# AdamBeedell/MLX8-WS-Audio-Transformer

Hardware: AMD Instinct MI355X
Metric: 4s@16kHz clips/sec through mel+Whisper-small encoder (higher is better)
Workload: dtype fp16; 1 GPU; int16 PCM [B,64000] in HBM -> Whisper log-mel [B,80,3000] -> Whisper-small encoder -> hidden [B,1500,768] fp32; mode=parity (clip zero-padded to 30 s, as the reference computes), precision=f16f8, fp16_exact_projection_matrices=0 of 48 (found by the library at upload), parallelism=dp1 (clip shards, no data-path collective)

## Files before the change

mlx8-ws-audio-transformer_amd/build.py:

```python
from __future__ import annotations

import os
import subprocess
import sys
from concurrent.futures import ThreadPoolExecutor

HERE = os.path.dirname(os.path.abspath(__file__))
CSRC = os.path.join(HERE, "csrc")
OBJ = os.path.join(CSRC, "_obj")
LIB = os.path.join(HERE, "libawt.so")
SOURCES = ["awt_api.hip", "logmel.hip", "gemm.hip", "attention.hip", "attention_f8.hip", "attention_bwd.hip", "elementwise.hip", "comm.hip", "decoder_ops.hip", "decoder_grad.hip", "bmm.hip", "decode_select.hip", "alignment.hip", "wgrad.hip", "cnn_ops.hip"]
HIPCC = os.environ.get("HIPCC", "/opt/rocm/bin/hipcc")
FLAGS = ["--offload-arch=gfx950", "-O3", "-std=c++20", "-fPIC", "-fno-gpu-rdc", "-Wall", "-Wno-unused-function"]


def _stale(target: str, deps) -> bool:
    if not os.path.exists(target):
        return True
    t = os.path.getmtime(target)
    return any(os.path.getmtime(d) > t for d in deps)


def _compile(src: str, force: bool) -> str:
    obj = os.path.join(OBJ, src.replace(".hip", ".o"))
    deps = [os.path.join(CSRC, src), os.path.join(CSRC, "common.h"), os.path.join(CSRC, "comm.h"), os.path.join(CSRC, "gemm_pp.h"), os.path.join(CSRC, "wgrad.h"), os.path.join(HERE, "..", "include", "awt.h")]
    if force or _stale(obj, deps):
        cmd = [HIPCC, *FLAGS, "-c", os.path.join(CSRC, src), "-o", obj]
        r = subprocess.run(cmd, capture_output=True, text=True)
        if r.returncode != 0:
            raise RuntimeError(f"hipcc failed for {src}:\n{r.stdout}\n{r.stderr}")
        if r.stderr.strip():
            sys.stderr.write(r.stderr)
    return obj


def build(force: bool = False, verbose: bool = True) -> str:
    os.makedirs(OBJ, exist_ok=True)
    with ThreadPoolExecutor(max_workers=min(len(SOURCES), os.cpu_count() or 4)) as ex:
        objs = list(ex.map(lambda s: _compile(s, force), SOURCES))
    if force or _stale(LIB, objs):
        cmd = [HIPCC, "--offload-arch=gfx950", "-shared", "-fPIC", "-o", LIB, *objs, "-ldl"]
        r = subprocess.run(cmd, capture_output=True, text=True)
        if r.returncode != 0:
            raise RuntimeError(f"link failed:\n{r.stdout}\n{r.stderr}")
    if verbose:
        print(f"built {LIB}")
    return LIB


if __name__ == "__main__":
    build(force="--force" in sys.argv)
```

mlx8-ws-audio-transformer_amd/csrc/awt_api.hip:

```cpp
#include <string.h>
#include <algorithm>
#include <string>
#include <vector>

#include "common.h"
#include "comm.h"
#include "wgrad.h"

static thread_local std::string g_err;
void awt_set_error(const std::string& msg) { g_err = msg; }
int awt_fail(int code, const std::string& msg) { g_err = msg; return code; }
extern "C" const char* awt_last_error(void) { return g_err.c_str(); }
extern "C" const char* awt_version(void) { return "awt 0.1 (gfx950)"; }

struct awt_prof_state {
  struct Span { hipEvent_t a, b; };
  std::vector<Span> spans[AWT_PROF_NCLASSES];
  std::vector<Span> pool;
  double flops[AWT_PROF_NCLASSES] = {};
  Span open[AWT_PROF_NCLASSES];
};

void awt_prof_begin(awt_ctx* c, int klass, hipStream_t s, double flops) {
  awt_prof_state* p = c->prof;
  awt_prof_state::Span sp;
  if (!p->pool.empty()) { sp = p->pool.back(); p->pool.pop_back(); }
  else { (void)hipEventCreate(&sp.a); (void)hipEventCreate(&sp.b); }
  (void)hipEventRecord(sp.a, s);
  p->open[klass] = sp;
  p->flops[klass] += flops;
}
void awt_prof_end(awt_ctx* c, int klass, hipStream_t s) {
  awt_prof_state* p = c->prof;
  (void)hipEventRecord(p->open[klass].b, s);
  p->spans[klass].push_back(p->open[klass]);
}

static int g_conv_live = 1;
static int g_pp_mask = 12;
extern "C" int awt_tuning_set(const char* key, int value) {
  AWT_REQUIRE(key, AWT_ERR_INVALID, "tuning_set: null key");
  if (!strcmp(key, "gemm_tile")) {
    AWT_REQUIRE(value == 0 || value == 64 || value == 128 || value == 256, AWT_ERR_INVALID, "tuning_set: gemm_tile must be 0 (auto), 64, 128 or 256");
    awt_gemm_force_tile(value);
    return AWT_OK;
  }
  if (!strcmp(key, "gemm_gm")) {
    AWT_REQUIRE(value >= 0 && value <= 64, AWT_ERR_INVALID, "tuning_set: gemm_gm must be 0 (default) .. 64");
    awt_gemm_set_gm(value);
    return AWT_OK;
  }
  if (!strcmp(key, "gemm_pp")) {
    AWT_REQUIRE(value >= 0 && value <= 2, AWT_ERR_INVALID, "tuning_set: gemm_pp must be 0 (off), 1 (automatic, default) or 2 (wherever supported)");
    awt_gemm_set_pp_mode(value);
    return AWT_OK;
  }
  if (!strcmp(key, "gemm_pp_mask")) {
    AWT_REQUIRE(value >= 0 && value <= 15, AWT_ERR_INVALID, "tuning_set: gemm_pp_mask is a bit set 0 .. 15 (1 qkv, 2 out_proj, 4 fc1, 8 fc2; fc2 only together with fc1)");
    g_pp_mask = value;
    return AWT_OK;
  }
  if (!strcmp(key, "gemm_mfma16")) {
    AWT_REQUIRE(value == 0 || value == 1, AWT_ERR_INVALID, "tuning_set: gemm_mfma16 must be 1 (default: the f16f8 GEMM's 16 x 16 MFMA form where it applies) or 0 (32 x 32 only)");
    awt_gemm_set_mfma16(value);
    return AWT_OK;
  }
  if (!strcmp(key, "conv_live")) {
    AWT_REQUIRE(value == 0 || value == 1, AWT_ERR_INVALID, "tuning_set: conv_live must be 1 (default: the conv stem of awt_audio_encode computes the live positions only) or 0 (every position)");
    g_conv_live = value;
    return AWT_OK;
  }
  if (!strcmp(key, "attn_shape")) {
    AWT_REQUIRE(value == 0 || (value >= 4 && value <= 6), AWT_ERR_INVALID, "tuning_set: attn_shape must be 0 (auto), 4, 5 or 6");
    awt_attn_force_shape(value);
    return AWT_OK;
  }
  if (!strcmp(key, "attn_qt")) {
    AWT_REQUIRE(value >= 0 && value <= 2, AWT_ERR_INVALID, "tuning_set: attn_qt must be 0 (auto), 1 or 2");
    awt_attn_force_qt(value);
    return AWT_OK;
  }
  AWT_REQUIRE(false, AWT_ERR_INVALID, "tuning_set: unknown key");
}

extern "C" int awt_prof_enable(awt_ctx* c, int on) {
  AWT_REQUIRE(c, AWT_ERR_INVALID, "prof_enable: null ctx");
  if (!c->prof) c->prof = new awt_prof_state();
  c->prof_on = on;
  return AWT_OK;
}
extern "C" int awt_prof_collect(awt_ctx* c, int klass, double* total_ms, int64_t* launches, double* flops) {
  AWT_REQUIRE(c && c->prof && klass >= 0 && klass < AWT_PROF_NCLASSES, AWT_ERR_INVALID, "prof_collect: bad argument");
  awt_prof_state* p = c->prof;
  double ms = 0;
  for (auto& sp : p->spans[klass]) {
    AWT_HIP_CHECK(hipEventSynchronize(sp.b));
    float t = 0;
    AWT_HIP_CHECK(hipEventElapsedTime(&t, sp.a, sp.b));
    ms += t;
    p->pool.push_back(sp);
  }
  if (total_ms) *total_ms = ms;
  if (launches) *launches = (int64_t)p->spans[klass].size();
  if (flops) *flops = p->flops[klass];
  p->spans[klass].clear();
  p->flops[klass] = 0;
  return AWT_OK;
}

extern "C" int awt_ctx_create(int device, awt_ctx** out) {
  AWT_REQUIRE(out, AWT_ERR_INVALID, "ctx_create: null out");
  int n = 0;
  AWT_HIP_CHECK(hipGetDeviceCount(&n));
  AWT_REQUIRE(device >= 0 && device < n, AWT_ERR_INVALID, "ctx_create: no such device");
  AWT_HIP_CHECK(hipSetDevice(device));
  hipDeviceProp_t prop;
  AWT_HIP_CHECK(hipGetDeviceProperties(&prop, device));
  AWT_REQUIRE(strncmp(prop.gcnArchName, "gfx950", 6) == 0, AWT_ERR_INVALID,
              std::string("libawt is built for gfx950 (MI355X) only; device is ") + prop.gcnArchName);
  awt_ctx* c = new awt_ctx();
  c->device = device;
  if (hipMalloc(&c->zeros, 256) != hipSuccess || hipMemset(c->zeros, 0, 256) != hipSuccess) {
    delete c;
    AWT_REQUIRE(false, AWT_ERR_HIP, "ctx_create: could not allocate the zero page");
  }
  int rc = logmel_prepare_impl(c, 400, 80, 0.0, 8000.0, 16000, 1);
  if (!rc) rc = logmel_prepare_impl(c, 400, 128, 0.0, 8000.0, 16000, 1);
  if (rc) { awt_ctx_destroy(c); return rc; }
  *out = c;
  return AWT_OK;
}
extern "C" int awt_logmel_prepare(awt_ctx* c, int n_fft, int n_mels, float f_min, float f_max, int sample_rate, int slaney) {
  return logmel_prepare_impl(c, n_fft, n_mels, (double)f_min, (double)f_max, sample_rate, slaney);
}
extern "C" int awt_resample_prepare(awt_ctx* c, int sr_in, int sr_out) { return resample_prepare_impl(c, sr_in, sr_out); }
extern "C" void awt_ctx_destroy(awt_ctx* c) {
  if (!c) return;
  awt_free_tables(c);
  if (c->zeros) (void)hipFree(c->zeros);
  if (c->prof) {
    for (int k = 0; k < AWT_PROF_NCLASSES; ++k)
      for (auto& sp : c->prof->spans[k]) { (void)hipEventDestroy(sp.a); (void)hipEventDestroy(sp.b); }
    for (auto& sp : c->prof->pool) { (void)hipEventDestroy(sp.a); (void)hipEventDestroy(sp.b); }
    delete c->prof;
  }
  delete c;
}

extern "C" int awt_logmel_whisper(awt_ctx* c, const void* pcm, int pcm_is_i16, int64_t pcm_stride, const int32_t* n_valid,
                                  int max_valid, int B, int n_frames_out, float* out, void* workspace, size_t ws_bytes,
                                  void* stream) {
  return logmel_whisper_impl(c, pcm, pcm_is_i16, pcm_stride, n_valid, max_valid, B, n_frames_out, 80, out, workspace, ws_bytes,
                             (hipStream_t)stream);
}
extern "C" int awt_logmel_whisper_mels(awt_ctx* c, const void* pcm, int pcm_is_i16, int64_t pcm_stride, const int32_t* n_valid,
                                       int max_valid, int B, int n_frames_out, int n_mels, float* out, void* workspace, size_t ws_bytes,
                                       void* stream) {
  return logmel_whisper_impl(c, pcm, pcm_is_i16, pcm_stride, n_valid, max_valid, B, n_frames_out, n_mels, out, workspace, ws_bytes,
                             (hipStream_t)stream);
}
extern "C" int awt_logmel_whisper_signal(awt_ctx* c, const void* pcm, int pcm_is_i16, int64_t pcm_stride, const int32_t* n_valid,
                                         int max_valid, int B, int n_signal, int n_mels, float* out, void* workspace, size_t ws_bytes,
                                         void* stream) {
  return logmel_whisper_impl(c, pcm, pcm_is_i16, pcm_stride, n_valid, max_valid, B, 0, n_mels, out, workspace, ws_bytes, (hipStream_t)stream,
                             n_signal);
}
extern "C" int awt_logmel_generic(awt_ctx* c, const float* pcm, int64_t pcm_stride, int B, int n_samples, int sample_rate,
                                  int n_fft, int hop, int n_mels, float f_min, float f_max, float log_eps, float* out,
                                  void* stream) {
  return logmel_generic_impl(c, pcm, pcm_stride, B, n_samples, sample_rate, n_fft, hop, n_mels, f_min, f_max, log_eps, out,
                             (hipStream_t)stream);
}

extern "C" int64_t awt_resampled_length(int n_in, int sr_in, int sr_out) {
  if (n_in <= 0 || sr_in <= 0 || sr_out <= 0) return 0;
  return resampled_length(n_in, sr_in, sr_out);
}
extern "C" int awt_prepare_waveform(awt_ctx* c, const void* pcm, int pcm_is_i16, int channels, int64_t channel_stride,
                                    int64_t sample_stride, int n_in, int sr_in, int sr_out, float* out, int n_out, void* stream) {
  return prepare_waveform_impl(c, pcm, pcm_is_i16, channels, channel_stride, sample_stride, n_in, sr_in, sr_out, out, n_out,
                               (hipStream_t)stream);
}

namespace {

struct Planes {
  bf16_t* hi = nullptr; bf16_t* lo = nullptr; uint8_t* x8 = nullptr; int64_t rows = 0, ld = 0;
  int* d_inexact = nullptr; bool exact16 = false;
  int64_t s_rows = 0;
  bf16_t* s16 = nullptr; uint8_t* s8 = nullptr;
  char* pp = nullptr;
};
struct Linear {
  Planes w; float* bias = nullptr; int N = 0, K = 0;
};
struct LoraGroup {
  bool active = false;
  Planes a;
  Planes b;
  Planes bT;
  Planes aT;
  int kp = 0;
};
struct Layer {
  Linear qkv, out, fc1, fc2;
  Planes qkvT, outT, fc1T, fc2T;
  Planes fc1T8, fc2T8;
  Planes fc1_8, fc2_8;
  float *ln1_g = nullptr, *ln1_b = nullptr, *ln2_g = nullptr, *ln2_b = nullptr;
  LoraGroup lq, lo_, l1, l2;
};

int conv1_k(int n_mels) { return (3 * n_mels + 63) / 64 * 64; }

}

struct awt_encoder {
  awt_ctx* ctx = nullptr;
  awt_encoder_cfg cfg{};
  int planes = 1;
  int prec = PREC_BF16X3;
  Linear conv1, conv2;
  float* pos = nullptr;
  float* zero_row = nullptr;
  float *lnf_g = nullptr, *lnf_b = nullptr;
  std::vector<Layer> layers;
  std::vector<void*> allocs;
  std::vector<std::string> seen;
  int chunk = 16;
  awt_comm* comm = nullptr;
  int comm_groups = 2;
  bool mlp_f8 = false;
  float* wt_tmp = nullptr;
  int grad_scale_log2 = 0;
  bool train_base = false;
  Planes conv2T[3];
  struct GradEntry { std::string name; size_t offset; int64_t shape[3]; int rank; };
  std::vector<GradEntry> glayout;
  size_t g_head = 0, g_per_layer = 0;
};

namespace {

int dev_alloc(awt_encoder* e, void** p, size_t bytes) {
  AWT_HIP_CHECK(hipMalloc(p, bytes));
  AWT_HIP_CHECK(hipMemset(*p, 0, bytes));
  e->allocs.push_back(*p);
  return AWT_OK;
}
int alloc_planes(awt_encoder* e, Planes* pl, int64_t rows, int64_t ld) {
  pl->rows = rows; pl->ld = ld;
  int rc = dev_alloc(e, (void**)&pl->hi, (size_t)rows * ld * 2); if (rc) return rc;
  if (e->planes == 2) { rc = dev_alloc(e, (void**)&pl->lo, (size_t)rows * ld * 2); if (rc) return rc; }
  if (e->prec == PREC_F16F8) {
    pl->x8 = (uint8_t*)pl->lo + (size_t)rows * ld;
    pl->s_rows = (rows + 255) / 256 * 256;
    rc = dev_alloc(e, (void**)&pl->s16, (size_t)pl->s_rows * ld * 2); if (rc) return rc;
    rc = dev_alloc(e, (void**)&pl->s8, (size_t)pl->s_rows * ld * 2); if (rc) return rc;
  }
  return AWT_OK;
}
int alloc_planes_f8(awt_encoder* e, Planes* pl, int64_t rows, int64_t ld) {
  pl->rows = rows; pl->ld = ld;
  int rc = dev_alloc(e, (void**)&pl->hi, (size_t)rows * ld * 2); if (rc) return rc;
  rc = dev_alloc(e, (void**)&pl->lo, (size_t)rows * ld * 2); if (rc) return rc;
  pl->x8 = (uint8_t*)pl->lo + (size_t)rows * ld;
  pl->s_rows = (rows + 255) / 256 * 256;
  rc = dev_alloc(e, (void**)&pl->s16, (size_t)pl->s_rows * ld * 2); if (rc) return rc;
  rc = dev_alloc(e, (void**)&pl->s8, (size_t)pl->s_rows * ld * 2); if (rc) return rc;
  return AWT_OK;
}
int alloc_linear(awt_encoder* e, Linear* l, int N, int K) {
  l->N = N; l->K = K;
  int rc = alloc_planes(e, &l->w, N, K); if (rc) return rc;
  return dev_alloc(e, (void**)&l->bias, (size_t)N * 4);
}
int alloc_lora(awt_encoder* e, LoraGroup* g, int slots, int K_in, int N_out) {
  g->active = true;
  g->kp = (int)(((int64_t)slots * e->cfg.lora_rank + 63) / 64 * 64);
  int rc = alloc_planes(e, &g->a, 128, K_in); if (rc) return rc;
  rc = alloc_planes(e, &g->b, N_out, g->kp); if (rc) return rc;
  if (e->cfg.training) {
    rc = alloc_planes(e, &g->bT, 128, N_out); if (rc) return rc;
    rc = alloc_planes(e, &g->aT, K_in, g->kp); if (rc) return rc;
  }
  return AWT_OK;
}

struct Workspace {
  float* x; bf16_t *ln[2], *qkv[2], *att[2], *ff[2], *u[2], *a1[2], *h1[2];
  size_t bytes;
};
// ... 30 lines not shown
Act act_offset(const Act& a, int64_t elems) {
  Act r;
  r.p16 = a.p16 + elems;
  r.lo16 = a.lo16 ? a.lo16 + elems : nullptr;
  r.hi8 = a.hi8 ? a.hi8 + elems : nullptr;
  r.lo8 = a.lo8 ? a.lo8 + elems : nullptr;
  return r;
}
void set_out(GemmOut& o, const Act& a) { o.hi = a.p16; o.lo = a.lo16; o.hi8 = a.hi8; o.lo8 = a.lo8; o.ilv = a.ilv; }
Act make_ilv(bf16_t* p0) { Act a; a.ilv = (char*)p0; return a; }

GemmSeg seg_plain(const Act& a, int64_t lda, const Planes& w, int64_t wcol, int K, int M) {
  GemmSeg s = gemm_seg_plain(a.p16, a.lo16, lda, w.hi, w.lo, (int)(w.ld / 32), (int)(wcol / 32), K, M);
  s.a8 = a.hi8; s.al8 = a.lo8; s.w8 = (const uint8_t*)w.lo; s.wl8 = w.x8;
  s.w_exact16 = w.exact16 ? 1 : 0;
  s.a_ilv = a.ilv; s.w_pp = w.pp;
  s.ws16 = w.s16; s.ws8 = w.s8; s.ws_rows = (int)w.s_rows;
  return s;
}
GemmSeg seg_plain(const bf16_t* a_hi, const bf16_t* a_lo, int64_t lda, const Planes& w, int64_t wcol, int K, int M) {
  Act a; a.p16 = const_cast<bf16_t*>(a_hi); a.lo16 = const_cast<bf16_t*>(a_lo);
  return seg_plain(a, lda, w, wcol, K, M);
}

int linear_with_lora(awt_encoder* e, bf16_t* const u[2], bf16_t* const in[2], int64_t ld_in, const Linear& lin, const LoraGroup& lg,
                     int M, GemmEpilogue epi, GemmOut out, hipStream_t s) {
  const int terms = e->prec;
  const Act ain = make_act(in[0], in[1], (size_t)M * ld_in, terms);
  GemmSeg segs[2];
  int nseg = 1;
  segs[0] = seg_plain(ain, ld_in, lin.w, 0, lin.K, M);
  if (lg.active) {
    GemmSeg us = seg_plain(ain, ld_in, lg.a, 0, lin.K, M);
    const Act au = make_act(u[0], u[1], (size_t)M * 128, terms);
    GemmOut uo{};
    set_out(uo, au); uo.ldo = lg.kp; uo.n_valid = lg.kp;
    uo.scale = e->cfg.lora_alpha / (float)e->cfg.lora_rank;
    int rc = launch_gemm(e->ctx, M, 128, &us, 1, terms, EPI_BF16, uo, s); if (rc) return rc;
    segs[1] = seg_plain(au, lg.kp, lg.b, 0, lg.kp, M);
    nseg = 2;
  }
  out.bias = lin.bias;
  out.n_valid = lin.N;
  return launch_gemm(e->ctx, M, lin.N, segs, nseg, terms, epi, out, s);
}

int linear_pp(awt_encoder* e, bf16_t* in0, const Linear& lin, int M, GemmEpilogue epi, GemmOut out, hipStream_t s) {
  GemmSeg sg = seg_plain(make_ilv(in0), lin.K, lin.w, 0, lin.K, M);
  out.bias = lin.bias;
  out.n_valid = lin.N;
  return launch_gemm_pp(e->ctx, M, lin.N, sg, epi, out, s);
}
bool use_pp(const awt_encoder* e, const Linear& lin, const LoraGroup& lg, int M, int epi) {
  const int mode = awt_gemm_pp_mode();
  if (mode == 0 || e->prec != PREC_F16F8 || !lin.w.pp || lg.active || !gemm_pp_supported(M, lin.N, lin.K, epi)) return false;
  if (mode == 2) return true;
  const int64_t t = (int64_t)((M + 255) / 256) * (lin.N / 256), c = gemm_pp_slots();
  return !lin.w.exact16 && c > 0 && t >= c && ((t + c - 1) / c) * c * 5 <= t * 6;
}

struct LayerBufs {
  float *x_in, *x_mid, *x_out;
  bf16_t *ln1[2], *qkv[2], *att[2], *ln2[2], *pre[2], *ff[2], *u[2];
  bf16_t *uo[2], *u1[2], *u2[2];
  float* lse;
};

struct TrainWs {
  std::vector<LayerBufs> layer;
  bf16_t *a1[2], *h1[2], *ff[2];
  bf16_t* pre1[2];
  float* x_final;
  float *dx_a, *dx_b, *dln, *delta, *partial;
  bf16_t *dxp[2], *dpre[2], *datt[2], *dqkv[2], *du[2];
  size_t partial_bytes, bytes;
};

TrainWs carve_train(const awt_encoder* e, char* base, int B) {
  const awt_encoder_cfg& c = e->cfg;
  const size_t P = e->planes, S = c.n_ctx, T = 2 * S, d = c.d_model, f = c.ffn_dim, H = c.n_heads;
  const size_t M = (size_t)B * S, Mt = (size_t)B * T;
  TrainWs w{};
  Carver cv(base);
  auto planes = [&](bf16_t* (&dst)[2], size_t elems) { dst[0] = dst[1] = nullptr; for (size_t p = 0; p < P; ++p) dst[p] = cv.take<bf16_t>(elems * 2); };
  w.layer.resize(c.n_layers);
  float* x = cv.take<float>(M * d * 4);
  for (int li = 0; li < c.n_layers; ++li) {
    LayerBufs& L = w.layer[li];
    L.x_in = x;
    L.x_mid = cv.take<float>(M * d * 4);
    L.x_out = cv.take<float>(M * d * 4);
    x = L.x_out;
    planes(L.ln1, M * d); planes(L.qkv, 3 * M * d); planes(L.att, M * d); planes(L.ln2, M * d); planes(L.pre, M * f);
    planes(L.u, M * 128);
    const bool has_o = e->layers[li].lo_.active, has_1 = e->layers[li].l1.active, has_2 = e->layers[li].l2.active;
    if (has_o) planes(L.uo, M * 128); else { L.uo[0] = L.u[0]; L.uo[1] = L.u[1]; }
    if (has_1) planes(L.u1, M * 128); else { L.u1[0] = L.u[0]; L.u1[1] = L.u[1]; }
    if (has_2) { planes(L.u2, M * 128); planes(L.ff, M * f); } else { L.u2[0] = L.u[0]; L.u2[1] = L.u[1]; L.ff[0] = L.ff[1] = nullptr; }
    if (e->train_base) planes(L.ff, M * f);
    L.lse = cv.take<float>((size_t)B * H * S * 4);
  }
  w.x_final = x;
  if (e->train_base) w.ff[0] = w.ff[1] = nullptr;
  else planes(w.ff, M * f);
  w.pre1[0] = w.pre1[1] = nullptr;
  if (e->train_base) { planes(w.a1, Mt * conv1_k(e->cfg.n_mels)); planes(w.h1, Mt * d); planes(w.pre1, Mt * d); }
  const size_t mark = cv.off;
  if (!e->train_base) { planes(w.a1, Mt * conv1_k(e->cfg.n_mels)); planes(w.h1, Mt * d); }
  const size_t conv_end = cv.off;
  cv.off = mark;
  w.dx_a = cv.take<float>(M * d * 4); w.dx_b = cv.take<float>(M * d * 4); w.dln = cv.take<float>(M * d * 4);
  w.delta = cv.take<float>((size_t)B * H * S * 4);
  planes(w.dxp, M * d); planes(w.dpre, M * f); planes(w.datt, M * d); planes(w.dqkv, 3 * M * d); planes(w.du, M * 128);
  w.partial_bytes = outer_reduce_partial_bytes((int)M, c.lora_rank > 0 ? c.lora_rank : 1, 1024);
  if (e->train_base) {
    const int Mi = (int)M, Mti = (int)Mt, di = (int)d, fi = (int)f;
    size_t pb = std::max({wgrad_partial_bytes(Mi, 3 * di, di), wgrad_partial_bytes(Mi, di, di), wgrad_partial_bytes(Mi, fi, di), wgrad_partial_bytes(Mi, di, fi),
                          wgrad_partial_bytes(Mti, di, c.n_mels), param_grad_partial_bytes(Mti, di)});
    w.partial_bytes = std::max(w.partial_bytes, pb);
  }
  w.partial = cv.take<float>(w.partial_bytes);
  w.bytes = std::max(cv.off, conv_end);
  for (int li = 0; li < c.n_layers; ++li) for (int p = 0; p < 2; ++p) if (!w.layer[li].ff[p]) w.layer[li].ff[p] = w.ff[p];
  return w;
}

int conv_stem(awt_encoder* e, const float* mel, int Bc, bf16_t* const a1[2], bf16_t* const h1[2], float* x, hipStream_t s, bf16_t* const* pre1 = nullptr,
              int Sc = 0, float* g = nullptr) {
  const awt_encoder_cfg& c = e->cfg;
  const int S = c.n_ctx, T = 2 * S, d = c.d_model, terms = e->prec;
  const bool compact = Sc > 0 && Sc < S && g && !pre1;
  const int So = compact ? Sc : S, To = 2 * So;
  const int M = Bc * So, Mt = Bc * To;
  const int k1 = conv1_k(c.n_mels);
  const Act aa1 = make_act(a1[0], a1[1], (size_t)Mt * k1, terms), ah1 = make_act(h1[0], h1[1], (size_t)Mt * d, terms);
  int rc = launch_im2col_conv1(e->ctx, mel, Bc, c.n_mels, T, To, k1, aa1, terms, s); if (rc) return rc;
  {
    GemmSeg sg = seg_plain(aa1, k1, e->conv1.w, 0, k1, Mt);
    GemmOut o{}; set_out(o, ah1); o.ldo = d; o.bias = e->conv1.bias; o.n_valid = d; o.m_pick = Bc * T;
    if (pre1) { o.hi2 = pre1[0]; o.lo2 = pre1[1]; }
    rc = launch_gemm(e->ctx, Mt, d, &sg, 1, terms, pre1 ? EPI_BF16_GELU_SAVE : EPI_BF16_GELU, o, s); if (rc) return rc;
  }
  GemmSeg sg[3];
  for (int dt = 0; dt < 3; ++dt) {
    sg[dt] = seg_plain(ah1, d, e->conv2.w, (int64_t)dt * d, d, M);
    sg[dt].rows_out = So; sg[dt].rows_in = To; sg[dt].row_mul = 2; sg[dt].row_add = dt - 1;
  }
  GemmOut o{}; o.f32 = compact ? g : x; o.ldo = d; o.bias = e->conv2.bias; o.n_valid = d; o.m_pick = Bc * S;
  if (compact) { o.pos = e->zero_row; o.rows_pos = 1; } else { o.pos = e->pos; o.rows_pos = S; }
  rc = launch_gemm(e->ctx, M, d, sg, 3, terms, EPI_F32_GELU_POS, o, s); if (rc || !compact) return rc;
  return launch_expand_conv_rows(e->ctx, g, e->pos, Bc, S, Sc, d, x, s);
}

int encoder_layer(awt_encoder* e, Layer& L, const LayerBufs& b, int Bc, bool save, hipStream_t s) {
  const awt_encoder_cfg& c = e->cfg;
  const int S = c.n_ctx, d = c.d_model, f = c.ffn_dim, H = c.n_heads, terms = e->prec;
  const int M = Bc * S;
  const int64_t plane = (int64_t)M * d;
  const bool pp_qkv = !save && (g_pp_mask & 1) && use_pp(e, L.qkv, L.lq, M, EPI_QKV), pp_out = !save && (g_pp_mask & 2) && use_pp(e, L.out, L.lo_, M, EPI_F32_RESID);
  const bool pp_fc1 = !save && (g_pp_mask & 4) && use_pp(e, L.fc1, L.l1, M, EPI_BF16_GELU), pp_fc2 = pp_fc1 && (g_pp_mask & 8) && use_pp(e, L.fc2, L.l2, M, EPI_F32_RESID);
  auto feeds = [&](Act a, const Linear& lin, const LoraGroup& lg) { if (terms == PREC_F16F8 && lin.w.exact16 && !lg.active) a.hi8 = nullptr; return a; };
  const Act aqkv = make_act(b.qkv[0], b.qkv[1], 3 * (size_t)plane, terms);
  const Act aatt = pp_out ? make_ilv(b.att[0]) : feeds(make_act(b.att[0], b.att[1], (size_t)plane, terms), L.out, L.lo_);
  int rc = launch_layernorm(e->ctx, b.x_in, L.ln1_g, L.ln1_b, M, d, 1e-5f, nullptr,
                            pp_qkv ? make_ilv(b.ln1[0]) : feeds(make_act(b.ln1[0], b.ln1[1], (size_t)plane, terms), L.qkv, L.lq), terms, s); if (rc) return rc;
  {
    GemmOut o{}; set_out(o, aqkv); o.scale = 0.125f * 1.4426950408889634f;
    o.S = S; o.H = H; o.plane_stride = plane;
    o.skip_v8 = terms == PREC_F16F8 && !attention_f16f8_reads_v8(save);
    rc = pp_qkv ? linear_pp(e, b.ln1[0], L.qkv, M, EPI_QKV, o, s) : linear_with_lora(e, b.u, b.ln1, d, L.qkv, L.lq, M, EPI_QKV, o, s);
    if (rc) return rc;
  }
  if (terms == PREC_F16F8) {
    const Act ak = act_offset(aqkv, plane), av = act_offset(aqkv, 2 * plane);
    rc = launch_attention_f16f8(e->ctx, F8Planes{aqkv.p16, aqkv.hi8, aqkv.lo8}, F8Planes{ak.p16, ak.hi8, ak.lo8}, F8Planes{av.p16, av.hi8, av.lo8},
                                F8Planes{aatt.p16, aatt.hi8, aatt.lo8}, nullptr, save ? b.lse : nullptr, Bc, H, S, s, aatt.ilv);
  } else {
    rc = launch_attention(e->ctx, b.qkv[0], b.qkv[1], b.qkv[0] + plane, b.qkv[1] ? b.qkv[1] + plane : nullptr, b.qkv[0] + 2 * plane,
                          b.qkv[1] ? b.qkv[1] + 2 * plane : nullptr, b.att[0], b.att[1], nullptr, save ? b.lse : nullptr, Bc, H, S, terms, s);
  }
  if (rc) return rc;
  {
    GemmOut o{}; o.f32 = b.x_mid; o.resid = b.x_in; o.ldo = d;
    rc = pp_out ? linear_pp(e, b.att[0], L.out, M, EPI_F32_RESID, o, s) : linear_with_lora(e, b.uo, b.att, d, L.out, L.lo_, M, EPI_F32_RESID, o, s);
    if (rc) return rc;
  }
  if (save && e->mlp_f8) {
    const Act aln2 = make_act(b.ln2[0], b.ln2[1], (size_t)plane, PREC_F16F8), aff = make_act(b.ff[0], b.ff[1], (size_t)M * f, PREC_F16F8);
    rc = launch_layernorm(e->ctx, b.x_mid, L.ln2_g, L.ln2_b, M, d, 1e-5f, nullptr, aln2, PREC_F16F8, s); if (rc) return rc;
    GemmSeg s1 = seg_plain(aln2, d, L.fc1_8, 0, d, M);
    GemmOut o1{}; set_out(o1, aff); o1.ldo = f; o1.n_valid = f; o1.bias = L.fc1.bias; o1.hi2 = b.pre[0]; o1.lo2 = b.pre[1]; o1.scale = 1.0f;
    rc = launch_gemm(e->ctx, M, f, &s1, 1, PREC_F16F8, EPI_BF16_GELU_SAVE, o1, s); if (rc) return rc;
    GemmSeg s2 = seg_plain(aff, f, L.fc2_8, 0, f, M);
    GemmOut o2{}; o2.f32 = b.x_out; o2.resid = b.x_mid; o2.ldo = d; o2.n_valid = d; o2.bias = L.fc2.bias;
    return launch_gemm(e->ctx, M, d, &s2, 1, PREC_F16F8, EPI_F32_RESID, o2, s);
  }
  rc = launch_layernorm(e->ctx, b.x_mid, L.ln2_g, L.ln2_b, M, d, 1e-5f, nullptr,
                        pp_fc1 ? make_ilv(b.ln2[0]) : feeds(make_act(b.ln2[0], b.ln2[1], (size_t)plane, terms), L.fc1, L.l1), terms, s); if (rc) return rc;
  {
    GemmOut o{}; set_out(o, pp_fc2 ? make_ilv(b.ff[0]) : feeds(make_act(b.ff[0], b.ff[1], (size_t)M * f, terms), L.fc2, L.l2)); o.ldo = f; o.hi2 = b.pre[0]; o.lo2 = b.pre[1];
    rc = pp_fc1 ? linear_pp(e, b.ln2[0], L.fc1, M, EPI_BF16_GELU, o, s)
                : linear_with_lora(e, b.u1, b.ln2, d, L.fc1, L.l1, M, save ? EPI_BF16_GELU_SAVE : EPI_BF16_GELU, o, s);
    if (rc) return rc;
  }
  GemmOut o{}; o.f32 = b.x_out; o.resid = b.x_mid; o.ldo = d;
  return pp_fc2 ? linear_pp(e, b.ff[0], L.fc2, M, EPI_F32_RESID, o, s) : linear_with_lora(e, b.u2, b.ff, f, L.fc2, L.l2, M, EPI_F32_RESID, o, s);
}

int forward_chunk(awt_encoder* e, const float* mel, int Bc, float* hidden, char* ws_base, hipStream_t s, int Sc = 0) {
  const awt_encoder_cfg& c = e->cfg;
  const int M = Bc * c.n_ctx, d = c.d_model;
  const bool two = e->planes == 2;
  Workspace w = carve(e, ws_base, Bc);
  bf16_t* a1[2] = {w.a1[0], two ? w.a1[1] : nullptr};
  bf16_t* h1[2] = {w.h1[0], two ? w.h1[1] : nullptr};
  float* g = nullptr;
  if (Sc > 0 && Sc < c.n_ctx) {
    char* const base = (char*)w.a1[0];
    const size_t room = (size_t)(ws_base + w.bytes - base), Mt = (size_t)Bc * 2 * Sc;
    Carver cv(base);
    bf16_t *ca1[2] = {nullptr, nullptr}, *ch1[2] = {nullptr, nullptr};
    for (int p = 0; p < e->planes; ++p) ca1[p] = cv.take<bf16_t>(Mt * conv1_k(c.n_mels) * 2);
    for (int p = 0; p < e->planes; ++p) ch1[p] = cv.take<bf16_t>(Mt * d * 2);
    float* cg = cv.take<float>((size_t)Bc * Sc * d * 4);
    if (cv.bytes() <= room) { g = cg; for (int p = 0; p < 2; ++p) { a1[p] = ca1[p]; h1[p] = ch1[p]; } }
  }
  int rc = conv_stem(e, mel, Bc, a1, h1, w.x, s, nullptr, g ? Sc : 0, g); if (rc) return rc;
  LayerBufs b{};
  b.x_in = b.x_mid = b.x_out = w.x;
  for (int p = 0; p < 2; ++p) {
    const bool on = p == 0 || two;
    b.ln1[p] = b.ln2[p] = on ? w.ln[p] : nullptr; b.qkv[p] = on ? w.qkv[p] : nullptr; b.att[p] = on ? w.att[p] : nullptr;
    b.ff[p] = on ? w.ff[p] : nullptr; b.u[p] = b.uo[p] = b.u1[p] = b.u2[p] = on ? w.u[p] : nullptr; b.pre[p] = nullptr;
  }
  for (int li = 0; li < c.n_layers; ++li) { rc = encoder_layer(e, e->layers[li], b, Bc, false, s); if (rc) return rc; }
  return launch_layernorm(e->ctx, w.x, e->lnf_g, e->lnf_b, M, d, 1e-5f, hidden, Act{}, e->prec, s);
}

bool parse_layer(const char* name, int* idx, const char** rest) {
  if (strncmp(name, "layers.", 7) != 0) return false;
  char* end = nullptr;
  long v = strtol(name + 7, &end, 10);
  if (end == name + 7 || *end != '.') return false;
  *idx = (int)v; *rest = end + 1;
  return true;
}

int check_shape(const char* name, const int64_t* shape, int rank, std::initializer_list<int64_t> want) {
  bool ok = rank == (int)want.size();
  int i = 0;
  for (int64_t w : want) { if (ok && shape[i] != w) ok = false; ++i; }
  if (!ok) {
    std::string m = std::string("set_weight: ") + name + " has shape [";
    for (int j = 0; j < rank; ++j) m += (j ? "," : "") + std::to_string(shape[j]);
    m += "], expected [";
    i = 0;
    for (int64_t w : want) m += (i++ ? "," : "") + std::to_string(w);
    return awt_fail(AWT_ERR_INVALID, m + "]");
  }
  return AWT_OK;
}

int copy_f32(float* dst, const float* src, size_t n, hipStream_t s) {
  AWT_HIP_CHECK(hipMemcpyAsync(dst, src, n * 4, hipMemcpyDeviceToDevice, s));
  return AWT_OK;
}

}

namespace {
void build_grad_layout(awt_encoder* e) {
  const awt_encoder_cfg& c = e->cfg;
  const int64_t d = c.d_model, f = c.ffn_dim;
  size_t off = 0;
  auto add = [&](const std::string& name, std::initializer_list<int64_t> shape) {
    awt_encoder::GradEntry g{name, off, {1, 1, 1}, (int)shape.size()};
    int i = 0; size_t n = 1;
    for (int64_t v : shape) { g.shape[i++] = v; n *= (size_t)v; }
    e->glayout.push_back(g);
    off += n;
  };
  add("conv1.weight", {d, c.n_mels, 3}); add("conv1.bias", {d}); add("conv2.weight", {d, d, 3}); add("conv2.bias", {d});
  add("layer_norm.weight", {d}); add("layer_norm.bias", {d});
  e->g_head = off;
  for (int li = 0; li < c.n_layers; ++li) {
    const std::string p = "layers." + std::to_string(li) + ".";
    add(p + "self_attn.q_proj.weight", {d, d}); add(p + "self_attn.k_proj.weight", {d, d}); add(p + "self_attn.v_proj.weight", {d, d});
    add(p + "self_attn.q_proj.bias", {d}); add(p + "self_attn.v_proj.bias", {d});
    add(p + "self_attn.out_proj.weight", {d, d}); add(p + "self_attn.out_proj.bias", {d});
    add(p + "self_attn_layer_norm.weight", {d}); add(p + "self_attn_layer_norm.bias", {d});
    add(p + "fc1.weight", {f, d}); add(p + "fc1.bias", {f}); add(p + "fc2.weight", {d, f}); add(p + "fc2.bias", {d});
    add(p + "final_layer_norm.weight", {d}); add(p + "final_layer_norm.bias", {d});
    if (li == 0) e->g_per_layer = off - e->g_head;
  }
}
}

extern "C" size_t awt_encoder_base_grad_count(const awt_encoder* e) {
  if (!e || !e->train_base) return 0;
  return e->g_head + (size_t)e->cfg.n_layers * e->g_per_layer;
}
extern "C" int awt_encoder_base_grad_params(const awt_encoder* e) { return (e && e->train_base) ? (int)e->glayout.size() : 0; }
extern "C" int awt_encoder_base_grad_param(const awt_encoder* e, int index, const char** name, size_t* offset, int64_t* shape, int* rank) {
  AWT_REQUIRE(e && e->train_base, AWT_ERR_STATE, "encoder_base_grad_param: encoder was not created with cfg.train_base");
  AWT_REQUIRE(index >= 0 && index < (int)e->glayout.size() && name && offset && shape && rank, AWT_ERR_INVALID, "encoder_base_grad_param: bad argument");
  const awt_encoder::GradEntry& g = e->glayout[index];
  *name = g.name.c_str(); *offset = g.offset; *rank = g.rank;
  for (int i = 0; i < 3; ++i) shape[i] = g.shape[i];
  return AWT_OK;
}

extern "C" int awt_encoder_create(awt_ctx* c, const awt_encoder_cfg* cfg, awt_encoder** out) {
  AWT_REQUIRE(c && cfg && out, AWT_ERR_INVALID, "encoder_create: null argument");
  AWT_REQUIRE(cfg->d_model > 0 && cfg->d_model % 128 == 0 && cfg->d_model <= 1280, AWT_ERR_INVALID, "encoder_create: d_model must be a multiple of 128, <= 1280");
  AWT_REQUIRE(cfg->n_heads > 0 && cfg->d_model == cfg->n_heads * 64, AWT_ERR_INVALID, "encoder_create: head_dim (d_model / n_heads) must be 64");
  AWT_REQUIRE(cfg->ffn_dim > 0 && cfg->ffn_dim % 128 == 0, AWT_ERR_INVALID, "encoder_create: ffn_dim must be a multiple of 128");
  AWT_REQUIRE(cfg->n_mels > 0 && cfg->n_mels % 8 == 0 && cfg->n_mels <= 128, AWT_ERR_INVALID, "encoder_create: n_mels must be a multiple of 8, <= 128");
  AWT_REQUIRE(cfg->n_layers > 0 && cfg->n_ctx > 0, AWT_ERR_INVALID, "encoder_create: n_layers and n_ctx must be positive");
  AWT_REQUIRE(prec_known(cfg->mfma_terms), AWT_ERR_INVALID,
              "encoder_create: mfma_terms must be 1 (bf16), 2 (fp16), 3 (bf16x3), 4 (fp16x3) or 5 (f16f8)");
  AWT_REQUIRE(!cfg->training || cfg->mfma_terms == PREC_BF16 || cfg->mfma_terms == PREC_BF16X3, AWT_ERR_INVALID,
              "encoder_create: training keeps its activations as bf16 planes: mfma_terms must be 1 or 3 (gradients do not fit fp16's range unscaled)");
  AWT_REQUIRE(cfg->backward_terms == 0 || cfg->backward_terms == cfg->mfma_terms || ((cfg->backward_terms == 1 || cfg->backward_terms == PREC_F16F8) && cfg->mfma_terms == 3),
              AWT_ERR_INVALID, "encoder_create: backward_terms must be 0 (= mfma_terms), mfma_terms, 1, or 5 (f16f8 MLP backward) with mfma_terms = 3");
  AWT_REQUIRE(cfg->backward_terms != PREC_F16F8 || (cfg->training && !(cfg->lora_targets & (AWT_LORA_FC1 | AWT_LORA_FC2))), AWT_ERR_INVALID,
              "encoder_create: backward_terms = 5 runs the MLP's backward GEMMs in f16f8: training mode, and no adapters on fc1 / fc2");
  AWT_REQUIRE(cfg->lora_rank >= 0 && cfg->lora_rank <= 32, AWT_ERR_INVALID, "encoder_create: lora_rank must be in 0..32");
  AWT_REQUIRE(cfg->lora_rank == 0 || cfg->lora_targets != 0, AWT_ERR_INVALID, "encoder_create: lora_rank > 0 needs lora_targets");
  AWT_REQUIRE(!cfg->training || cfg->lora_rank > 0 || cfg->train_base, AWT_ERR_INVALID, "encoder_create: training mode needs adapters (lora_rank > 0) or train_base");
  AWT_REQUIRE(!cfg->train_base || cfg->training, AWT_ERR_INVALID, "encoder_create: train_base needs training mode");
  AWT_REQUIRE(!cfg->train_base || cfg->lora_rank == 0, AWT_ERR_INVALID, "encoder_create: train_base trains the base weights themselves: no adapters in this mode (lora_rank must be 0)");
  AWT_REQUIRE(!cfg->train_base || cfg->backward_terms != PREC_F16F8, AWT_ERR_INVALID,
              "encoder_create: train_base forms its weight gradients from bf16 planes: backward_terms = 5 (f16f8 MLP backward) is not available in this mode");
  awt_encoder* e = new awt_encoder();
  e->ctx = c; e->cfg = *cfg; e->prec = cfg->mfma_terms; e->planes = (cfg->mfma_terms == PREC_BF16 || cfg->mfma_terms == PREC_F16) ? 1 : 2;
  e->chunk = cfg->chunk_clips > 0 ? cfg->chunk_clips : 64;
  e->mlp_f8 = cfg->backward_terms == PREC_F16F8;
  e->train_base = cfg->train_base != 0;
  const int d = cfg->d_model, f = cfg->ffn_dim;
  int rc = alloc_linear(e, &e->conv1, d, conv1_k(cfg->n_mels));
  if (!rc && e->mlp_f8) rc = dev_alloc(e, (void**)&e->wt_tmp, (size_t)f * d * 4);
  if (!rc && e->train_base) rc = dev_alloc(e, (void**)&e->wt_tmp, (size_t)d * d * 4);
  for (int dt = 0; dt < 3 && !rc && e->train_base; ++dt) rc = alloc_planes(e, &e->conv2T[dt], d, d);
  if (!rc) rc = alloc_linear(e, &e->conv2, d, 3 * d);
  if (!rc) rc = dev_alloc(e, (void**)&e->pos, (size_t)cfg->n_ctx * d * 4);
  if (!rc) rc = dev_alloc(e, (void**)&e->zero_row, (size_t)d * 4);
  if (!rc) rc = dev_alloc(e, (void**)&e->lnf_g, (size_t)d * 4);
  if (!rc) rc = dev_alloc(e, (void**)&e->lnf_b, (size_t)d * 4);
  e->layers.resize(cfg->n_layers);
  const bool lora = cfg->lora_rank > 0;
  for (int i = 0; i < cfg->n_layers && !rc; ++i) {
    Layer& L = e->layers[i];
    rc = alloc_linear(e, &L.qkv, 3 * d, d);
    if (!rc) rc = alloc_linear(e, &L.out, d, d);
    if (!rc) rc = alloc_linear(e, &L.fc1, f, d);
    if (!rc) rc = alloc_linear(e, &L.fc2, d, f);
    if ((e->prec == PREC_F16F8 || e->prec == PREC_F16X3) && !cfg->training)
      for (Linear* lin : {&L.qkv, &L.out, &L.fc1, &L.fc2}) if (!rc) rc = dev_alloc(e, (void**)&lin->w.d_inexact, 4 * sizeof(int));
    if (e->prec == PREC_F16F8 && !cfg->training)
      for (Linear* lin : {&L.qkv, &L.out, &L.fc1, &L.fc2})
        if (!rc && lin->N % 256 == 0 && lin->K % 64 == 0 && lin->K >= 128) rc = dev_alloc(e, (void**)&lin->w.pp, gemm_pp_weight_bytes(lin->N, lin->K));
    if (cfg->training) {
      if (!rc) rc = alloc_planes(e, &L.qkvT, d, 3 * d);
      if (!rc) rc = alloc_planes(e, &L.outT, d, d);
      if (!rc) rc = alloc_planes(e, &L.fc1T, d, f);
      if (!rc) rc = alloc_planes(e, &L.fc2T, f, d);
      if (!rc && e->mlp_f8) rc = alloc_planes_f8(e, &L.fc1T8, d, f);
      if (!rc && e->mlp_f8) rc = alloc_planes_f8(e, &L.fc2T8, f, d);
      if (!rc && e->mlp_f8) rc = alloc_planes_f8(e, &L.fc1_8, f, d);
      if (!rc && e->mlp_f8) rc = alloc_planes_f8(e, &L.fc2_8, d, f);
    }
    float** lnp[4] = {&L.ln1_g, &L.ln1_b, &L.ln2_g, &L.ln2_b};
    for (int k = 0; k < 4 && !rc; ++k) rc = dev_alloc(e, (void**)lnp[k], (size_t)d * 4);
    if (lora && !rc && (cfg->lora_targets & (AWT_LORA_Q | AWT_LORA_K | AWT_LORA_V))) rc = alloc_lora(e, &L.lq, 3, d, 3 * d);
    if (lora && !rc && (cfg->lora_targets & AWT_LORA_OUT)) rc = alloc_lora(e, &L.lo_, 1, d, d);
    if (lora && !rc && (cfg->lora_targets & AWT_LORA_FC1)) rc = alloc_lora(e, &L.l1, 1, d, f);
    if (lora && !rc && (cfg->lora_targets & AWT_LORA_FC2)) rc = alloc_lora(e, &L.l2, 1, f, d);
  }
  if (rc) { awt_encoder_destroy(e); return rc; }
  if (e->train_base) build_grad_layout(e);
  *out = e;
  return AWT_OK;
}

extern "C" void awt_encoder_destroy(awt_encoder* e) {
  if (!e) return;
  for (void* p : e->allocs) (void)hipFree(p);
  delete e;
// ... 546 lines not shown
```

mlx8-ws-audio-transformer_amd/csrc/common.h:

```cpp
#pragma once
#include <hip/hip_runtime.h>
#include <stdint.h>
#include <string>

#include "../../include/awt.h"

typedef unsigned short bf16_t;
typedef short bf16x8 __attribute__((ext_vector_type(8)));
typedef short bf16x4 __attribute__((ext_vector_type(4)));
typedef float f32x4 __attribute__((ext_vector_type(4)));
typedef float f32x16 __attribute__((ext_vector_type(16)));
typedef double f64x4 __attribute__((ext_vector_type(4)));

typedef _Float16 f16x8 __attribute__((ext_vector_type(8)));
typedef int i32x8 __attribute__((ext_vector_type(8)));
typedef int i32x2 __attribute__((ext_vector_type(2)));

#define AWT_WAVE 64

enum { PREC_BF16 = 1, PREC_F16 = 2, PREC_BF16X3 = 3, PREC_F16X3 = 4, PREC_F16F8 = 5 };
__host__ __device__ constexpr bool prec_known(int p) { return p >= PREC_BF16 && p <= PREC_F16F8; }
__host__ __device__ constexpr bool prec_is_f16(int p) { return p == PREC_F16 || p == PREC_F16X3 || p == PREC_F16F8; }
__host__ __device__ constexpr int prec_products(int p) { return (p == PREC_BF16 || p == PREC_F16) ? 1 : 3; }
constexpr int kF8Act = -2;
// ... 74 lines not shown
  h16 = make_uint2(pack2(h[0], h[1]), pack2(h[2], h[3]));
  hi8 = fp8x4<S>(v[0], v[1], v[2], v[3]);
  lo8 = fp8x4<S + kF8Lo>(l[0], l[1], l[2], l[3]);
}

__device__ __forceinline__ void glds16_asm(const void* gsrc, char* lds_wave_base) {
  const unsigned dst = __builtin_amdgcn_readfirstlane((unsigned)(uintptr_t)(__attribute__((address_space(3))) char*)lds_wave_base);
  unsigned keep;
  asm volatile("s_mov_b32 %0, m0\n\ts_mov_b32 m0, %2\n\ts_nop 0\n\tglobal_load_lds_dwordx4 %1, off\n\ts_mov_b32 m0, %0"
               : "=&s"(keep) : "v"(gsrc), "s"(dst) : "memory");
}

__device__ __forceinline__ void glds16_asm_sbase(const void* sbase, unsigned lane_byte_off, unsigned lds_wave_addr) {
  const unsigned dst = __builtin_amdgcn_readfirstlane(lds_wave_addr);
  unsigned keep;
  asm volatile("s_mov_b32 %0, m0\n\ts_mov_b32 m0, %3\n\ts_nop 0\n\tglobal_load_lds_dwordx4 %1, %2\n\ts_mov_b32 m0, %0"
               : "=&s"(keep) : "v"(lane_byte_off), "s"(sbase), "s"(dst) : "memory");
}

__device__ __forceinline__ float erf_fast(float x) {
  const float ax = fabsf(x);
  const float t = __builtin_amdgcn_rcpf(fmaf(0.3275911f, ax, 1.0f));
  float p = fmaf(1.061405429f, t, -1.453152027f);
  p = fmaf(p, t, 1.421413741f);
  p = fmaf(p, t, -0.284496736f);
  p = fmaf(p, t, 0.254829592f);
  const float y = 1.0f - p * t * __expf(-ax * ax);
  return copysignf(y, x);
}
__device__ __forceinline__ float gelu_erf(float x) {
  const float t = fabsf(x) * 0.70710678118654752440f, tc = fminf(t, 4.2f);
  float q = fmaf(-0.00010022104106610641f, tc, 0.0004615735961124301f);
  q = fmaf(q, tc, 0.0023022345267236233f);
  q = fmaf(q, tc, -0.029452508315443993f);
  q = fmaf(q, tc, 0.14896366000175476f);
  q = fmaf(q, tc, 0.9183286428451538f);
  q = fmaf(q, tc, 1.6279137134552002f);
  const float e = __builtin_amdgcn_exp2f(fmaf(tc - t, 12.5f, -tc * q));
  const float h = 0.5f * x;
  return fmaf(-fabsf(h), e, h + fabsf(h));
}

__host__ __device__ __forceinline__ int64_t w_frag_index(int n, int k, int ksteps) {
  const int nt = n >> 4, r = n & 15, ks = k >> 5, kq = (k & 31) >> 3, j = k & 7;
  return (((int64_t)nt * ksteps + ks) * 64 + (kq * 16 + r)) * 8 + j;
}

__host__ __device__ __forceinline__ int64_t w16f8_index(int n, int k, int ksteps16) {
  const int nt = n >> 5, r = n & 31, ks = k >> 4, h = (k & 15) >> 3, j = k & 7;
  return (((int64_t)nt * ksteps16 + ks) * 64 + (h * 32 + r)) * 8 + j;
}
__host__ __device__ __forceinline__ int64_t w8_index(int n, int k, int ktiles64) {
  const int nt = n >> 5, r = n & 31, kt = k >> 6, h = (k & 63) >> 5, b = k & 31;
  return (((int64_t)nt * ktiles64 + kt) * 64 + (h * 32 + r)) * 32 + b;
}

__host__ __device__ __forceinline__ int64_t w8s_index(int n, int k, int ktiles64, int is_hi8) {
  const int nt = n >> 4, r = n & 15, kt = k >> 6, kb = ((k & 63) >> 5) + (is_hi8 ? 2 : 0), b = k & 31;
  return (((int64_t)nt * ktiles64 + kt) * 64 + (kb * 16 + r)) * 32 + b;
}

struct Act { bf16_t* p16 = nullptr; bf16_t* lo16 = nullptr; uint8_t* hi8 = nullptr; uint8_t* lo8 = nullptr; char* ilv = nullptr; };
__device__ __forceinline__ void store_ilv4(char* ilv, int64_t off, uint2 h16, unsigned hi8, unsigned lo8) {
  char* line = ilv + (off >> 6) * 256;
  const int e = (int)(off & 63);
  *reinterpret_cast<uint2*>(line + e * 2) = h16;
  *reinterpret_cast<unsigned*>(line + 128 + e) = hi8;
  *reinterpret_cast<unsigned*>(line + 192 + e) = lo8;
}
template <int PREC, int S = kF8Act, bool SAT = false>
__device__ __forceinline__ void store_act4(const Act& o, int64_t off, const float (&v)[4]) {
  if constexpr (PREC == PREC_F16F8) {
    uint2 h16; unsigned hi8, lo8;
    f16f8x4<S, SAT>(v, h16, hi8, lo8);
    if (o.ilv) { store_ilv4(o.ilv, off, h16, hi8, lo8); return; }
    *reinterpret_cast<uint2*>(o.p16 + off) = h16;
    if (o.hi8) *reinterpret_cast<unsigned*>(o.hi8 + off) = hi8;
    *reinterpret_cast<unsigned*>(o.lo8 + off) = lo8;
  } else {
    bf16_t h[4], l[4];
#pragma unroll
    for (int t = 0; t < 4; ++t) split16<PREC == PREC_F16X3>(v[t], h[t], l[t]);
    *reinterpret_cast<uint2*>(o.p16 + off) = make_uint2(pack2(h[0], h[1]), pack2(h[2], h[3]));
    if (o.lo16) *reinterpret_cast<uint2*>(o.lo16 + off) = make_uint2(pack2(l[0], l[1]), pack2(l[2], l[3]));
  }
}

__device__ __forceinline__ float wave_max(float x) {
#pragma unroll
  for (int o = 32; o > 0; o >>= 1) x = fmaxf(x, __shfl_xor(x, o));
  return x;
}
__device__ __forceinline__ float wave_sum(float x) {
#pragma unroll
  for (int o = 32; o > 0; o >>= 1) x += __shfl_xor(x, o);
  return x;
}

template <class I>
__device__ __forceinline__ int xcd_contiguous(I block, int n) {
  const int xcd = block & 7, idx = block >> 3;
  const int q = n >> 3, r = n & 7;
  return (xcd < r ? xcd * (q + 1) : r * (q + 1) + (xcd - r) * q) + idx;
}
__device__ __forceinline__ void gemm_tile_coords(int tile, int tiles_m, int tiles_n, int GM, int& tm, int& tn) {
  const int grp = tile / (GM * tiles_n);
  const int gm = min(GM, tiles_m - grp * GM);
  const int within = tile - grp * GM * tiles_n;
  tn = within / gm; tm = grp * GM + (within - tn * gm);
}
__device__ __forceinline__ bool row_map_source(int m, int rows_out, int rows_in, int row_mul, int row_add, int64_t& src) {
  const int grp = m / rows_out, r = m - grp * rows_out;
  const int sr = r * row_mul + row_add;
  const bool ok = sr >= 0 && sr < rows_in;
  src = (int64_t)grp * rows_in + sr;
  return ok;
}

void awt_set_error(const std::string& msg);
int awt_fail(int code, const std::string& msg);

#define AWT_HIP_CHECK(expr)                                                                      \
  do {                                                                                           \
    hipError_t _e = (expr);                                                                      \
    if (_e != hipSuccess)                                                                        \
      return awt_fail(AWT_ERR_HIP, std::string(#expr) + ": " + hipGetErrorString(_e));           \
  } while (0)

#define AWT_REQUIRE(cond, code, msg)         \
  do {                                       \
    if (!(cond)) return awt_fail(code, msg); \
  } while (0)

inline size_t align_up(size_t x) { return (x + 255) & ~(size_t)255; }
struct Carver {
  char* base; size_t off = 0;
  explicit Carver(void* b) : base((char*)b) {}
  template <class T = char> T* take(size_t bytes) { char* p = base ? base + off : nullptr; off += align_up(bytes); return (T*)p; }
  size_t bytes() const { return off; }
};
struct PlanePair { bf16_t *hi, *lo; };
inline PlanePair take_planes(Carver& cv, size_t elems) { return {cv.take<bf16_t>(elems * 2), cv.take<bf16_t>(elems * 2)}; }
struct PlanesWs { PlanePair p; size_t bytes; };
inline PlanesWs planes_layout(void* base, size_t elems) { Carver cv(base); return {take_planes(cv, elems), cv.bytes()}; }

struct awt_prof_state;
struct awt_ctx {
  int device = 0;
  int prof_on = 0;
  awt_prof_state* prof = nullptr;
  struct Table;
  Table* tables = nullptr;
  void* zeros = nullptr;
};

#define AWT_ONCE_PER_DEVICE(set)                                   \
  do {                                                             \
    static unsigned long long _done = 0;                           \
    int _dev = 0;                                                  \
    AWT_HIP_CHECK(hipGetDevice(&_dev));                            \
    if (!((_done >> (_dev & 63)) & 1ull)) {                        \
      set;                                                         \
      _done |= 1ull << (_dev & 63);                                \
    }                                                              \
  } while (0)

template <auto Kernel, class... Args>
int launch_kernel(dim3 grid, dim3 block, int lds, hipStream_t s, const Args&... args) {
  AWT_ONCE_PER_DEVICE(AWT_HIP_CHECK(hipFuncSetAttribute((const void*)Kernel, hipFuncAttributeMaxDynamicSharedMemorySize, lds)));
  hipLaunchKernelGGL(Kernel, grid, block, lds, s, args...);
  AWT_HIP_CHECK(hipGetLastError());
  return AWT_OK;
}

void awt_prof_begin(awt_ctx* c, int klass, hipStream_t s, double flops);
void awt_prof_end(awt_ctx* c, int klass, hipStream_t s);

struct ProfScope {
  awt_ctx* c; int klass; hipStream_t s;
  ProfScope(awt_ctx* c_, int k, hipStream_t s_, double flops = 0.0) : c(c_), klass(k), s(s_) {
    if (c && (c->prof_on >> klass) & 1) awt_prof_begin(c, klass, s, flops);
  }
  ~ProfScope() { if (c && (c->prof_on >> klass) & 1) awt_prof_end(c, klass, s); }
};

struct GemmSeg {
  const bf16_t* a_hi; const bf16_t* a_lo; int64_t lda;
  const bf16_t* w_hi; const bf16_t* w_lo; int w_ksteps, w_k0;
  const uint8_t* a8; const uint8_t* al8; const uint8_t* w8; const uint8_t* wl8;
  int w_exact16;
  const char* a_ilv; const char* w_pp;
  const bf16_t* ws16; const uint8_t* ws8;
  int ws_rows;
  int K;
  int rows_out, rows_in, row_mul, row_add;
};

inline GemmSeg gemm_seg_plain(const bf16_t* a_hi, const bf16_t* a_lo, int64_t lda, const bf16_t* w_hi, const bf16_t* w_lo, int w_ksteps, int w_k0, int K, int M) {
  GemmSeg s{};
  s.a_hi = a_hi; s.a_lo = a_lo; s.lda = lda; s.w_hi = w_hi; s.w_lo = w_lo; s.w_ksteps = w_ksteps; s.w_k0 = w_k0; s.K = K;
  s.rows_out = M; s.rows_in = M; s.row_mul = 1; s.row_add = 0;
  return s;
}

enum GemmEpilogue {
  EPI_F32 = 0,
  EPI_F32_RESID = 1,
  EPI_BF16 = 2,
  EPI_BF16_GELU = 3,
  EPI_QKV = 4,
  EPI_F32_GELU_POS = 5,
  EPI_BF16_GELU_SAVE = 6,
  EPI_BF16_DGELU = 7
};

struct GemmOut {
  float* f32; const float* resid; int64_t ldo;
  bf16_t* hi; bf16_t* lo;
  uint8_t* hi8; uint8_t* lo8;
  char* ilv;
  bf16_t* hi2; bf16_t* lo2;
  const bf16_t* pre_hi; const bf16_t* pre_lo;
  const float* bias;
  const float* pos; int rows_pos;
  float scale;
  int n_valid;
  int S, H;
  int64_t plane_stride;
  int skip_v8;
  int m_pick;
};

int launch_gemm(awt_ctx* c, int M, int N, const GemmSeg* segs, int nseg, int prec, GemmEpilogue epi, const GemmOut& out,
                hipStream_t s);
bool gemm_pp_supported(int M, int N, int K, int epi);
int gemm_pp_slots();
int launch_gemm_pp(awt_ctx* c, int M, int N, const GemmSeg& seg, GemmEpilogue epi, const GemmOut& out, hipStream_t s);
size_t gemm_pp_weight_bytes(int N, int K);
int launch_pack_weight_pp(awt_ctx* c, const float* src, int N, int K, int row_off, char* dst, hipStream_t s);
int awt_gemm_pp_mode();
void awt_gemm_set_pp_mode(int v);
void awt_gemm_set_mfma16(int v);

int launch_layernorm(awt_ctx* c, const float* x, const float* gamma, const float* beta, int M, int d, float eps,
                     float* out_f32, const Act& out, int prec, hipStream_t s);
int launch_attention(awt_ctx* c, const bf16_t* q_hi, const bf16_t* q_lo, const bf16_t* k_hi, const bf16_t* k_lo,
                     const bf16_t* v_hi, const bf16_t* v_lo, bf16_t* o_hi, bf16_t* o_lo, float* o_f32, float* lse, int B, int H,
                     int S, int terms, hipStream_t s);
int launch_split_f32(awt_ctx* c, const float* x, int64_t n, float scale, bf16_t* hi, bf16_t* lo, hipStream_t s);
struct F8Planes { bf16_t* p16; uint8_t* hi8; uint8_t* lo8; };
int launch_split_planes(awt_ctx* c, const float* x, int64_t n, float scale, int prec, int f8_exp, bf16_t* p16, bf16_t* lo16, uint8_t* hi8,
                        uint8_t* lo8, hipStream_t s, char* ilv = nullptr);
int launch_attention_f16f8(awt_ctx* c, const F8Planes& q, const F8Planes& k, const F8Planes& v, const F8Planes& o, float* o_f32,
                           float* lse, int B, int H, int S, hipStream_t s, char* o_ilv = nullptr);
int launch_pack_weight(awt_ctx* c, const float* src, int N, int C, int taps, int64_t ld, int row_off, int col_off, float scale,
                       bf16_t* hi, bf16_t* lo, uint8_t* lo8, int prec, hipStream_t s, int* inexact = nullptr,
                       bf16_t* s16 = nullptr, uint8_t* s8 = nullptr);
int launch_im2col_conv1(awt_ctx* c, const float* mel, int B, int C, int T_mel, int T, int K_dst, const Act& out, int prec, hipStream_t s);
int launch_expand_conv_rows(awt_ctx* c, const float* g, const float* pos, int B, int S, int Sc, int d, float* x, hipStream_t s);
int conv_stem_positions(int n_ctx, int max_valid);

int logmel_whisper_impl(awt_ctx* c, const void* pcm, int pcm_is_i16, int64_t pcm_stride, const int32_t* n_valid,
                        int max_valid, int B, int n_frames_out, int n_mels, float* out, void* workspace, size_t ws_bytes, hipStream_t s,
                        int n_signal = 0);
int logmel_generic_impl(awt_ctx* c, const float* pcm, int64_t pcm_stride, int B, int n_samples, int sample_rate, int n_fft,
                        int hop, int n_mels, float f_min, float f_max, float log_eps, float* out, hipStream_t s);
int prepare_waveform_impl(awt_ctx* c, const void* pcm, int pcm_is_i16, int channels, int64_t channel_stride, int64_t sample_stride,
                          int n_in, int sr_in, int sr_out, float* out, int n_out, hipStream_t s);
int64_t resampled_length(int n_in, int sr_in, int sr_out);
int logmel_prepare_impl(awt_ctx* c, int n_fft, int n_mels, double f_min, double f_max, int sample_rate, int slaney);
int resample_prepare_impl(awt_ctx* c, int sr_in, int sr_out);
void awt_free_tables(awt_ctx* c);
void awt_attn_force_shape(int v);
void awt_attn_force_qt(int v);
void awt_gemm_set_gm(int v);
bool attention_f16f8_reads_v8(bool with_lse);
void awt_gemm_force_tile(int t);

int launch_attention_bwd(awt_ctx* c, const bf16_t* q_hi, const bf16_t* q_lo, const bf16_t* k_hi, const bf16_t* k_lo,
                         const bf16_t* v_hi, const bf16_t* v_lo, const bf16_t* o_hi, const bf16_t* o_lo, const bf16_t* do_hi,
                         const bf16_t* do_lo, const float* lse2, float* delta, bf16_t* g_hi, bf16_t* g_lo, int B, int H, int S,
                         float qscale, int terms, int grad_terms, hipStream_t s);
int launch_layernorm_bwd(awt_ctx* c, const float* dy, const float* x, const float* gamma, const float* dres, int M, int d, float eps,
                         float* dx, bf16_t* dx_hi, bf16_t* dx_lo, hipStream_t s, float gscale = 1.0f, const Act* out8 = nullptr);
int launch_transpose_f32(awt_ctx* c, const float* src, int N, int C, float* dst, hipStream_t s);
int launch_pack_weight_t(awt_ctx* c, const float* src, int N, int C, int64_t ld, int row_off, int col_off, float scale, bf16_t* hi,
                         bf16_t* lo, hipStream_t s);
int launch_outer_reduce(awt_ctx* c, const bf16_t* x_hi, const bf16_t* x_lo, int64_t ldx, int xcol, int r, const bf16_t* y_hi,
                        const bf16_t* y_lo, int64_t ldy, int ycol, int ny, int M, float scale, float* out, int64_t sj, int64_t sn,
                        float* partial, size_t partial_bytes, int accumulate, hipStream_t s);
size_t outer_reduce_partial_bytes(int M, int r, int ny);
```

mlx8-ws-audio-transformer_amd/csrc/elementwise.hip:

```cpp
#include "common.h"
#include "gemm_pp.h"

namespace {

__device__ __forceinline__ float4 ldg_once(const float4* p) {
  const f32x4 t = __builtin_nontemporal_load(reinterpret_cast<const f32x4*>(p));
  return make_float4(t[0], t[1], t[2], t[3]);
}

constexpr int kLnMaxChunks = 5;

template <int PREC>
__global__ __launch_bounds__(256) void layernorm_kernel(const float* __restrict__ x, const float* __restrict__ gamma,
                                                        const float* __restrict__ beta, int M, int d, float eps,
                                                        float* out_f32, Act out) {
  const int lane = threadIdx.x & 63;
  const int row = blockIdx.x * 4 + (threadIdx.x >> 6);
  if (row >= M) return;
  const int nchunk = d >> 2;
  const float4* xr = reinterpret_cast<const float4*>(x + (int64_t)row * d);
  float4 v[kLnMaxChunks];
  float sum = 0.f;
#pragma unroll
  for (int i = 0; i < kLnMaxChunks; ++i) {
    const int c = lane + 64 * i;
    if (c < nchunk) v[i] = ldg_once(xr + c);
    else v[i] = make_float4(0.f, 0.f, 0.f, 0.f);
    sum += (v[i].x + v[i].y) + (v[i].z + v[i].w);
  }
#pragma unroll
  for (int o = 32; o > 0; o >>= 1) sum += __shfl_xor(sum, o);
  const float mean = sum / (float)d;
  float sq = 0.f;
#pragma unroll
  for (int i = 0; i < kLnMaxChunks; ++i) {
    const int c = lane + 64 * i;
    if (c < nchunk) {
      const float a = v[i].x - mean, b = v[i].y - mean, cc = v[i].z - mean, dd = v[i].w - mean;
      sq += (a * a + b * b) + (cc * cc + dd * dd);
    }
  }
#pragma unroll
  for (int o = 32; o > 0; o >>= 1) sq += __shfl_xor(sq, o);
  const float rstd = 1.0f / sqrtf(sq / (float)d + eps);
  const float4* g4 = reinterpret_cast<const float4*>(gamma);
  const float4* b4 = reinterpret_cast<const float4*>(beta);
#pragma unroll
  for (int i = 0; i < kLnMaxChunks; ++i) {
    const int c = lane + 64 * i;
    if (c >= nchunk) continue;
    const float4 g = g4[c], bb = b4[c];
    float y[4] = {(v[i].x - mean) * rstd * g.x + bb.x, (v[i].y - mean) * rstd * g.y + bb.y,
                  (v[i].z - mean) * rstd * g.z + bb.z, (v[i].w - mean) * rstd * g.w + bb.w};
    if (out_f32) reinterpret_cast<float4*>(out_f32 + (int64_t)row * d)[c] = make_float4(y[0], y[1], y[2], y[3]);
    else store_act4<PREC>(out, (int64_t)row * d + 4 * c, y);
  }
}

__global__ __launch_bounds__(256) void split_kernel(const float* __restrict__ x, int64_t n4, float scale, bf16_t* hi, bf16_t* lo) {
  for (int64_t i = (int64_t)blockIdx.x * blockDim.x + threadIdx.x; i < n4; i += (int64_t)gridDim.x * blockDim.x) {
    const float4 v = reinterpret_cast<const float4*>(x)[i];
    bf16_t h[4], l[4];
    split_bf16(v.x * scale, h[0], l[0]); split_bf16(v.y * scale, h[1], l[1]); split_bf16(v.z * scale, h[2], l[2]); split_bf16(v.w * scale, h[3], l[3]);
    reinterpret_cast<uint2*>(hi)[i] = make_uint2(pack2(h[0], h[1]), pack2(h[2], h[3]));
    if (lo) reinterpret_cast<uint2*>(lo)[i] = make_uint2(pack2(l[0], l[1]), pack2(l[2], l[3]));
  }
}

template <int PREC>
__global__ __launch_bounds__(256) void split_planes_kernel(const float* __restrict__ x, int64_t n4, float scale, float f8_scale, bf16_t* p16,
                                                           bf16_t* lo16, uint8_t* hi8, uint8_t* lo8, char* ilv) {
  for (int64_t i = (int64_t)blockIdx.x * blockDim.x + threadIdx.x; i < n4; i += (int64_t)gridDim.x * blockDim.x) {
    const float4 q = reinterpret_cast<const float4*>(x)[i];
    const float v[4] = {q.x * scale, q.y * scale, q.z * scale, q.w * scale};
    bf16_t h[4], l[4];
    if constexpr (PREC == PREC_F16F8) {
      float lo[4];
#pragma unroll
      for (int t = 0; t < 4; ++t) { h[t] = f32_to_f16(v[t]); lo[t] = (v[t] - f16_to_f32(h[t])) * (f8_scale * pow2f(kF8Lo)); }
      const uint2 h16 = make_uint2(pack2(h[0], h[1]), pack2(h[2], h[3]));
      const unsigned b_hi = fp8x4<0>(v[0] * f8_scale, v[1] * f8_scale, v[2] * f8_scale, v[3] * f8_scale), b_lo = fp8x4<0>(lo[0], lo[1], lo[2], lo[3]);
      if (ilv) { store_ilv4(ilv, i * 4, h16, b_hi, b_lo); continue; }
      reinterpret_cast<uint2*>(p16)[i] = h16;
      reinterpret_cast<unsigned*>(hi8)[i] = b_hi;
      reinterpret_cast<unsigned*>(lo8)[i] = b_lo;
    } else {
#pragma unroll
      for (int t = 0; t < 4; ++t) split16<PREC == PREC_F16X3>(v[t], h[t], l[t]);
      reinterpret_cast<uint2*>(p16)[i] = make_uint2(pack2(h[0], h[1]), pack2(h[2], h[3]));
      if (lo16) reinterpret_cast<uint2*>(lo16)[i] = make_uint2(pack2(l[0], l[1]), pack2(l[2], l[3]));
    }
  }
}

template <int PREC>
__global__ __launch_bounds__(256) void pack_weight_kernel(const float* __restrict__ src, int N, int C, int taps, int64_t ld,
                                                          int row_off, int col_off, float scale, bf16_t* hi, bf16_t* lo, uint8_t* lo8,
                                                          int* inexact, bf16_t* s16, uint8_t* s8) {
  const int K = C * taps;
  bool any_inexact = false;
  const int64_t total = (int64_t)N * K;
  for (int64_t i = (int64_t)blockIdx.x * blockDim.x + threadIdx.x; i < total; i += (int64_t)gridDim.x * blockDim.x) {
    const int n = (int)(i / K), k = (int)(i - (int64_t)n * K);
    const int dt = k / C, c = k - dt * C;
    const float v = src[((int64_t)n * C + c) * taps + dt] * scale;
    if constexpr (PREC == PREC_F16F8) {
      const bf16_t h = f32_to_f16(v);
      hi[w16f8_index(row_off + n, col_off + k, (int)(ld >> 4))] = h;
      const int64_t o8 = w8_index(row_off + n, col_off + k, (int)(ld >> 6));
      reinterpret_cast<uint8_t*>(lo)[o8] = (uint8_t)(fp8x4<kF8Wgt>(v, 0.f, 0.f, 0.f) & 0xFF);
      lo8[o8] = (uint8_t)(fp8x4<kF8Wgt + kF8Lo>(v - f16_to_f32(h), 0.f, 0.f, 0.f) & 0xFF);
      if (s16) {
        s16[w_frag_index(row_off + n, col_off + k, (int)(ld >> 5))] = h;
        s8[w8s_index(row_off + n, col_off + k, (int)(ld >> 6), 1)] = reinterpret_cast<uint8_t*>(lo)[o8];
        s8[w8s_index(row_off + n, col_off + k, (int)(ld >> 6), 0)] = lo8[o8];
      }
      any_inexact |= (v != f16_to_f32(h));
    } else {
      bf16_t h, l; split16<PREC == PREC_F16X3>(v, h, l);
      if (PREC == PREC_F16X3) any_inexact |= ((l & 0x7FFF) != 0);
      const int64_t o = w_frag_index(row_off + n, col_off + k, (int)(ld >> 5));
      hi[o] = h;
      if (lo) lo[o] = l;
    }
  }
  if ((PREC == PREC_F16F8 || PREC == PREC_F16X3) && inexact && __builtin_amdgcn_ballot_w64(any_inexact) != 0 && (threadIdx.x & 63) == 0) atomicOr(inexact, 1);
}

__global__ __launch_bounds__(256) void pack_weight_pp_kernel(const float* __restrict__ src, int N, int K, int row_off, char* dst) {
  const int nk = K >> 5;
  const int64_t total = (int64_t)N * (K >> 2);
  for (int64_t i = (int64_t)blockIdx.x * blockDim.x + threadIdx.x; i < total; i += (int64_t)gridDim.x * blockDim.x) {
    const int n = (int)(i / (K >> 2)), k = (int)(i - (int64_t)n * (K >> 2)) * 4;
    const float4 q = *reinterpret_cast<const float4*>(src + (int64_t)n * K + k);
    const float v[4] = {q.x, q.y, q.z, q.w};
    uint2 h16; unsigned hi8, lo8;
    f16f8x4<kF8Wgt>(v, h16, hi8, lo8);
    const int row = row_off + n, bn = row >> 8, nin = row & 255, sgrp = (nin >> 5) & 1, grp = k >> 6, e = k & 63;
    char* rx = dst + pp::w_region_offset(bn, 2 * grp, sgrp, nk);
    char* ry = dst + pp::w_region_offset(bn, 2 * grp + 1, sgrp, nk);
    *reinterpret_cast<uint2*>(rx + pp::w_row_offset(nin, e >> 3) + (e & 7) * 2) = h16;
    *reinterpret_cast<unsigned*>(ry + pp::w_row_offset(nin, e >> 4) + (e & 15)) = lo8;
    *reinterpret_cast<unsigned*>(ry + pp::w_row_offset(nin, 4 + (e >> 4)) + (e & 15)) = hi8;
  }
}

constexpr int kImTile = 64;
template <int PREC>
__global__ __launch_bounds__(256) void im2col_conv1_kernel(const float* __restrict__ mel, int C, int T_mel, int T, int K_dst, Act out) {
  extern __shared__ __attribute__((aligned(16))) char smem[];
  float* tile = reinterpret_cast<float*>(smem);
  const int pitch = kImTile + 3;
  const int b = blockIdx.y, t0 = blockIdx.x * kImTile;
  const float* mb = mel + (int64_t)b * C * T_mel;
  for (int i = threadIdx.x; i < C * (kImTile + 2); i += 256) {
    const int c = i / (kImTile + 2), tt = i - c * (kImTile + 2);
    const int t = t0 + tt - 1;
    tile[c * pitch + tt] = (t >= 0 && t < T) ? mb[(int64_t)c * T_mel + t] : 0.f;
  }
  __syncthreads();
  const int groups = K_dst / 8;
  const int cg = C / 8;
  for (int i = threadIdx.x; i < kImTile * groups; i += 256) {
    const int tl = i / groups, g = i - tl * groups;
    const int t = t0 + tl;
    if (t >= T) continue;
    const int dt = g / cg, c0 = (g - dt * cg) * 8;
    float v[2][4];
#pragma unroll
    for (int j = 0; j < 8; ++j) v[j >> 2][j & 3] = dt < 3 ? tile[(c0 + j) * pitch + tl + dt] : 0.f;
    const int64_t off = ((int64_t)b * T + t) * K_dst + g * 8;
    store_act4<PREC>(out, off, v[0]);
    store_act4<PREC>(out, off + 4, v[1]);
  }
}

__global__ __launch_bounds__(256) void expand_conv_rows_kernel(const float4* __restrict__ g, const float4* __restrict__ pos, int rows, int S, int Sc, int d4,
                                                                float4* __restrict__ x) {
  const int lane = threadIdx.x & 63;
  const int row = blockIdx.x * 4 + (threadIdx.x >> 6);
  if (row >= rows) return;
  const int b = row / S, p = row - b * S;
  const int src = p < Sc - 1 ? p : (p == S - 1 ? Sc - 1 : Sc - 2);
  const float4* gr = g + ((int64_t)b * Sc + src) * d4;
  const float4* pr = pos + (int64_t)p * d4;
  float4* xr = x + (int64_t)row * d4;
  float4 v[kLnMaxChunks], q[kLnMaxChunks];
#pragma unroll
  for (int i = 0; i < kLnMaxChunks; ++i) {
    const int c = lane + 64 * i;
    if (c < d4) { v[i] = gr[c]; q[i] = pr[c]; }
  }
#pragma unroll
  for (int i = 0; i < kLnMaxChunks; ++i) {
    const int c = lane + 64 * i;
    if (c < d4) xr[c] = make_float4(v[i].x + q[i].x, v[i].y + q[i].y, v[i].z + q[i].z, v[i].w + q[i].w);
  }
}

__global__ __launch_bounds__(256) void layernorm_bwd_kernel(const float* __restrict__ dy, const float* __restrict__ x,
                                                            const float* __restrict__ gamma, const float* dres, int M, int d,
                                                            float eps, float* dx, bf16_t* dx_hi, bf16_t* dx_lo, float gscale, Act out8) {
  const int lane = threadIdx.x & 63;
  const int row = blockIdx.x * 4 + (threadIdx.x >> 6);
  if (row >= M) return;
  const int nchunk = d >> 2;
  const float4* xr = reinterpret_cast<const float4*>(x + (int64_t)row * d);
  const float4* dyr = reinterpret_cast<const float4*>(dy + (int64_t)row * d);
  const float4* g4 = reinterpret_cast<const float4*>(gamma);
// ... 333 lines not shown
```

mlx8-ws-audio-transformer_amd/csrc/gemm.hip:

```cpp
#include <algorithm>
#include <type_traits>
#include "common.h"
#include "gemm_pp.h"

#ifndef AWT_GEMM_GM
#define AWT_GEMM_GM 8
#endif

namespace {

int g_gm = AWT_GEMM_GM;
constexpr int kMaxSeg = 3;
typedef int i32x4_t __attribute__((ext_vector_type(4)));

struct GemmArgs {
  int M, N, nseg, tiles_m, tiles_n;
  int gm;
  GemmSeg seg[kMaxSeg];
  GemmOut out;
  const bf16_t* zeros;
  int64_t bs_a, bs_w, bs_o;
};

struct Cfg64 { static constexpr int WM = 2, WN = 2, TM = 2, TN = 4; };
struct Cfg128 { static constexpr int WM = 2, WN = 2, TM = 4, TN = 4; };
struct CfgW4 { static constexpr int WM = 1, WN = 4, TM = 8, TN = 4; };

template <int BK> __device__ __forceinline__ int swz(int row);
template <> __device__ __forceinline__ int swz<64>(int row) { return (row >> 1) & 7; }
template <> __device__ __forceinline__ int swz<32>(int row) { return (0x1320 >> (((row >> 2) & 3) * 4)) & 3; }

template <int TERMS, int BK, class CFG, bool WX = false>
struct Tile {
  static constexpr int BM = CFG::WM * CFG::TM * 16, BN = CFG::WN * CFG::TN * 16;
  static constexpr int THREADS = CFG::WM * CFG::WN * 64;
  static constexpr int NP = (TERMS == 3) ? 2 : 1;
  static constexpr int PLANE_A = BM * BK * 2;
  static constexpr int STAGE = NP * PLANE_A;
  static constexpr int CPR = BK / 8;
  static constexpr int ITERS_A = (BM * CPR) / THREADS;
  static constexpr int KS = BK / 32;
  static constexpr int NA = NP * ITERS_A;
  static constexpr int NPW = WX ? 1 : NP;
  static constexpr int NB = NPW * KS * CFG::TN;
  static constexpr int LDS_BYTES = (2 * STAGE > CFG::WM * CFG::WN * 16 * 68 * 4) ? 2 * STAGE : CFG::WM * CFG::WN * 16 * 68 * 4;
};

__device__ __forceinline__ void glds16(const void* gsrc, char* lds_wave_base) {
  __builtin_amdgcn_global_load_lds((const __attribute__((address_space(1))) void*)gsrc,
                                   (__attribute__((address_space(3))) void*)lds_wave_base, 16, 0, 0);
}

template <int TERMS, int BK, class CFG, bool WX = false>
struct Stager {
  using T = Tile<TERMS, BK, CFG, WX>;
  const bf16_t* a_hi[T::ITERS_A]; const bf16_t* a_lo[T::ITERS_A];
  const bf16_t* w_hi; const bf16_t* w_lo;
  int64_t w_tile_stride;
  int64_t za = 0, zw = 0;
  int si, kk, nk;

  __device__ __forceinline__ void open_segment(const GemmArgs& g, int seg, int m0, int n0, int wc, int wave, int lane) {
    si = seg; kk = 0;
    const GemmSeg& sg = g.seg[seg];
    nk = sg.K / BK;
#pragma unroll
    for (int it = 0; it < T::ITERS_A; ++it) {
      const int p = it * T::THREADS + wave * 64 + lane;
      const int row = p / T::CPR;
      const int c = (p % T::CPR) ^ swz<BK>(row);
      int m = m0 + row; m = m < g.M ? m : g.M - 1;
      int64_t src;
      const bool ok = row_map_source(m, sg.rows_out, sg.rows_in, sg.row_mul, sg.row_add, src);
      const int64_t aoff = src * sg.lda + c * 8 + za;
      a_hi[it] = ok ? sg.a_hi + aoff : nullptr;
      a_lo[it] = (ok && TERMS == 3) ? sg.a_lo + aoff : nullptr;
    }
    w_tile_stride = (int64_t)sg.w_ksteps * 512;
    const int nt0 = (n0 >> 4) + wc * CFG::TN;
    const int64_t woff = ((int64_t)nt0 * sg.w_ksteps + sg.w_k0) * 512 + lane * 8 + zw;
    w_hi = sg.w_hi + woff;
    w_lo = (TERMS == 3) ? sg.w_lo + woff : nullptr;
  }
  template <int OP>
  __device__ __forceinline__ void issue(const GemmArgs& g, char* stage_base, int wave, bf16x8 (&nbh)[T::KS][CFG::TN], bf16x8 (&nbl)[T::KS][CFG::TN]) {
    static_assert(OP >= 0 && OP < T::NA + T::NB, "operation index");
    if constexpr (OP < T::NA) {
      constexpr int plane = OP % T::NP, it = OP / T::NP;
      char* dst = stage_base + (it * T::THREADS + wave * 64) * 16 + plane * T::PLANE_A;
      const bf16_t* src = plane == 0 ? a_hi[it] : a_lo[it];
      glds16(src ? (const void*)(src + kk * BK) : (const void*)g.zeros, dst);
    } else {
      constexpr int q = OP - T::NA;
      constexpr int plane = q % T::NPW, r = q / T::NPW, j = r % CFG::TN, ks = r / CFG::TN;
      const int64_t off = (int64_t)j * w_tile_stride + (int64_t)(kk * T::KS + ks) * 512;
      if (plane == 0) nbh[ks][j] = *reinterpret_cast<const bf16x8*>(w_hi + off);
      else nbl[ks][j] = *reinterpret_cast<const bf16x8*>(w_lo + off);
    }
  }
  __device__ __forceinline__ void advance(const GemmArgs& g, int m0, int n0, int wc, int wave, int lane) {
    if (++kk == nk && si + 1 < g.nseg) open_segment(g, si + 1, m0, n0, wc, wave, lane);
  }
};

template <int EPI, bool FULL = false>
__device__ __forceinline__ float4 load_side4(const GemmOut& o, int m, int n, int M) {
  float4 r = make_float4(0.f, 0.f, 0.f, 0.f);
  if constexpr (!FULL) { if (m >= M || n >= o.n_valid) return r; }
  if (EPI == EPI_F32_RESID) {
    r = *reinterpret_cast<const float4*>(o.resid + (int64_t)m * o.ldo + n);
  } else if (EPI == EPI_F32_GELU_POS) {
    r = *reinterpret_cast<const float4*>(o.pos + (int64_t)(m % o.rows_pos) * o.ldo + n);
  } else if (EPI == EPI_BF16_DGELU) {
    const int64_t off = (int64_t)m * o.ldo + n;
    const uint2 ph = *reinterpret_cast<const uint2*>(o.pre_hi + off);
    uint2 pl = make_uint2(0u, 0u);
    if (o.pre_lo) pl = *reinterpret_cast<const uint2*>(o.pre_lo + off);
    r.x = bf16_to_f32((bf16_t)(ph.x & 0xFFFF)) + bf16_to_f32((bf16_t)(pl.x & 0xFFFF));
    r.y = bf16_to_f32((bf16_t)(ph.x >> 16)) + bf16_to_f32((bf16_t)(pl.x >> 16));
    r.z = bf16_to_f32((bf16_t)(ph.y & 0xFFFF)) + bf16_to_f32((bf16_t)(pl.y & 0xFFFF));
    r.w = bf16_to_f32((bf16_t)(ph.y >> 16)) + bf16_to_f32((bf16_t)(pl.y >> 16));
  }
  return r;
}

template <int EPI, bool F16, bool FULL>
__device__ __forceinline__ void store_out4(const GemmOut& o, int m, int n, float4 acc, float4 side, float4 b, int M) {
  if constexpr (!FULL) { if (m >= M || n >= o.n_valid) return; }
  float v[4] = {acc.x, acc.y, acc.z, acc.w};
  const float sd[4] = {side.x, side.y, side.z, side.w};
  v[0] += b.x; v[1] += b.y; v[2] += b.z; v[3] += b.w;
  if (EPI == EPI_F32 || EPI == EPI_F32_RESID || EPI == EPI_F32_GELU_POS) {
    float* dst = o.f32 + (int64_t)m * o.ldo + n;
    if (EPI == EPI_F32_RESID) {
#pragma unroll
      for (int t = 0; t < 4; ++t) v[t] += sd[t];
    } else if (EPI == EPI_F32_GELU_POS) {
#pragma unroll
      for (int t = 0; t < 4; ++t) v[t] = gelu_erf(v[t]) + sd[t];
    }
    *reinterpret_cast<float4*>(dst) = make_float4(v[0], v[1], v[2], v[3]);
  } else {
    int64_t off;
    if (EPI == EPI_QKV) {
      const int d = o.H * 64;
      const int which = n / d, within = n - which * d;
      const int h = within >> 6, e = within & 63;
      const int b = m / o.S, s = m - b * o.S;
      if (which == 0) { v[0] *= o.scale; v[1] *= o.scale; v[2] *= o.scale; v[3] *= o.scale; }
      off = (int64_t)which * o.plane_stride + (((int64_t)b * o.H + h) * o.S + s) * 64 + e;
    } else {
      off = (int64_t)m * o.ldo + n;
      if (EPI == EPI_BF16_GELU_SAVE) {
        bf16_t ph[4], pl[4];
#pragma unroll
        for (int t = 0; t < 4; ++t) split_bf16(v[t], ph[t], pl[t]);
        *reinterpret_cast<uint2*>(o.hi2 + off) = make_uint2(pack2(ph[0], ph[1]), pack2(ph[2], ph[3]));
        if (o.lo2) *reinterpret_cast<uint2*>(o.lo2 + off) = make_uint2(pack2(pl[0], pl[1]), pack2(pl[2], pl[3]));
      }
      if (EPI == EPI_BF16_DGELU) {
#pragma unroll
        for (int t = 0; t < 4; ++t) {
          const float x = sd[t];
          v[t] *= 0.5f * (1.0f + erf_fast(x * 0.70710678118654752440f)) + x * 0.39894228040143267794f * __expf(-0.5f * x * x);
        }
      } else {
#pragma unroll
        for (int t = 0; t < 4; ++t) v[t] = (EPI == EPI_BF16_GELU || EPI == EPI_BF16_GELU_SAVE) ? gelu_erf(v[t]) : v[t] * o.scale;
      }
    }
    bf16_t hi[4], lo[4];
#pragma unroll
    for (int t = 0; t < 4; ++t) split16<F16>(v[t], hi[t], lo[t]);
    *reinterpret_cast<uint2*>(o.hi + off) = make_uint2(pack2(hi[0], hi[1]), pack2(hi[2], hi[3]));
    if (o.lo) *reinterpret_cast<uint2*>(o.lo + off) = make_uint2(pack2(lo[0], lo[1]), pack2(lo[2], lo[3]));
  }
}

template <int EPI, bool FULL, bool ILV = false>
__device__ __forceinline__ void store_out8_f8(const GemmOut& o, int m, int n, float4 acc0, float4 acc1, float4 side0, float4 side1, float4 b0, float4 b1, int M) {
  if constexpr (!FULL) { if (m >= M || n >= o.n_valid) return; }
  float v[8] = {acc0.x, acc0.y, acc0.z, acc0.w, acc1.x, acc1.y, acc1.z, acc1.w};
  const float sd[8] = {side0.x, side0.y, side0.z, side0.w, side1.x, side1.y, side1.z, side1.w};
  v[0] += b0.x; v[1] += b0.y; v[2] += b0.z; v[3] += b0.w; v[4] += b1.x; v[5] += b1.y; v[6] += b1.z; v[7] += b1.w;
  if (EPI == EPI_F32 || EPI == EPI_F32_RESID || EPI == EPI_F32_GELU_POS) {
    float* dst = o.f32 + (int64_t)m * o.ldo + n;
#pragma unroll
    for (int t = 0; t < 8; ++t) v[t] = EPI == EPI_F32_RESID ? v[t] + sd[t] : (EPI == EPI_F32_GELU_POS ? gelu_erf(v[t]) + sd[t] : v[t]);
    *reinterpret_cast<float4*>(dst) = make_float4(v[0], v[1], v[2], v[3]);
    *reinterpret_cast<float4*>(dst + 4) = make_float4(v[4], v[5], v[6], v[7]);
    return;
  }
  int64_t off;
  float inv8 = pow2f(-kF8Act), lim8 = 448.0f * pow2f(-kF8Act);
  if (EPI == EPI_QKV) {
    const int d = o.H * 64;
    const int which = n / d, within = n - which * d;
    inv8 = which == 0 ? pow2f(-kF8Q) : pow2f(-kF8KV); lim8 = which == 0 ? 448.0f * pow2f(-kF8Q) : 448.0f * pow2f(-kF8KV);
    const int h = within >> 6, e = within & 63;
    const int b = m / o.S, s = m - b * o.S;
    if (which == 0) {
#pragma unroll
      for (int t = 0; t < 8; ++t) v[t] *= o.scale;
    }
    off = (int64_t)which * o.plane_stride + (((int64_t)b * o.H + h) * o.S + s) * 64 + e;
  } else {
    off = (int64_t)m * o.ldo + n;
    if constexpr (EPI == EPI_BF16_GELU_SAVE) {
      bf16_t ph[8], pl[8];
#pragma unroll
      for (int t = 0; t < 8; ++t) split_bf16(v[t], ph[t], pl[t]);
      *reinterpret_cast<uint4*>(o.hi2 + off) = make_uint4(pack2(ph[0], ph[1]), pack2(ph[2], ph[3]), pack2(ph[4], ph[5]), pack2(ph[6], ph[7]));
      if (o.lo2) *reinterpret_cast<uint4*>(o.lo2 + off) = make_uint4(pack2(pl[0], pl[1]), pack2(pl[2], pl[3]), pack2(pl[4], pl[5]), pack2(pl[6], pl[7]));
#pragma unroll
      for (int t = 0; t < 8; ++t) v[t] = gelu_erf(v[t]);
    } else if constexpr (EPI == EPI_BF16_DGELU) {
#pragma unroll
      for (int t = 0; t < 8; ++t) {
        const float x = sd[t];
        v[t] *= 0.5f * (1.0f + erf_fast(x * 0.70710678118654752440f)) + x * 0.39894228040143267794f * __expf(-0.5f * x * x);
        v[t] = __builtin_amdgcn_fmed3f(v[t], -kF16Max, kF16Max);
      }
    } else {
#pragma unroll
      for (int t = 0; t < 8; ++t) v[t] = EPI == EPI_BF16_GELU ? gelu_erf(v[t]) : v[t] * o.scale;
    }
  }
  const float invl8 = inv8 * pow2f(-kF8Lo), liml8 = lim8 * pow2f(-kF8Lo);
  bf16_t h[8]; float l[8];
#pragma unroll
  for (int t = 0; t < 8; ++t) { h[t] = f32_to_f16(v[t]); l[t] = v[t] - f16_to_f32(h[t]); }
  if constexpr (ILV) {
    char* line = o.ilv + (off >> 6) * 256;
    const int e = (int)(off & 63);
    __builtin_nontemporal_store((i32x4_t){(int)pack2(h[0], h[1]), (int)pack2(h[2], h[3]), (int)pack2(h[4], h[5]), (int)pack2(h[6], h[7])}, reinterpret_cast<i32x4_t*>(line + e * 2));
    __builtin_nontemporal_store((i32x2){(int)fp8x4_rt(v[0], v[1], v[2], v[3], lim8, inv8), (int)fp8x4_rt(v[4], v[5], v[6], v[7], lim8, inv8)}, reinterpret_cast<i32x2*>(line + 128 + e));
    __builtin_nontemporal_store((i32x2){(int)fp8x4_rt(l[0], l[1], l[2], l[3], liml8, invl8), (int)fp8x4_rt(l[4], l[5], l[6], l[7], liml8, invl8)}, reinterpret_cast<i32x2*>(line + 192 + e));
    return;
  }
  __builtin_nontemporal_store((i32x4_t){(int)pack2(h[0], h[1]), (int)pack2(h[2], h[3]), (int)pack2(h[4], h[5]), (int)pack2(h[6], h[7])}, reinterpret_cast<i32x4_t*>(o.hi + off));
  if (EPI == EPI_QKV && o.skip_v8 && n >= 2 * o.H * 64) return;
  if (o.hi8) __builtin_nontemporal_store((i32x2){(int)fp8x4_rt(v[0], v[1], v[2], v[3], lim8, inv8), (int)fp8x4_rt(v[4], v[5], v[6], v[7], lim8, inv8)}, reinterpret_cast<i32x2*>(o.hi8 + off));
  __builtin_nontemporal_store((i32x2){(int)fp8x4_rt(l[0], l[1], l[2], l[3], liml8, invl8), (int)fp8x4_rt(l[4], l[5], l[6], l[7], liml8, invl8)}, reinterpret_cast<i32x2*>(o.lo8 + off));
}

template <int TERMS, int BK, int EPI, class CFG, bool F16, bool WX = false, bool BATCH = false>
__global__ __launch_bounds__(CFG::WM * CFG::WN * 64, 2) void gemm_kernel(GemmArgs g) {
  static_assert(!BATCH || EPI == EPI_F32 || EPI == EPI_F32_RESID, "batched launches write fp32 matrices");
  static_assert(!WX || TERMS == 3, "the exact-weight form belongs to the split product");
  using T = Tile<TERMS, BK, CFG, WX>;
  using ST = Stager<TERMS, BK, CFG, WX>;
  constexpr int TM = CFG::TM, TN = CFG::TN, KS = T::KS, STEPS = KS * TM, NOPS = T::NA + T::NB;
  constexpr int OPS_PER_STEP = (NOPS + STEPS - 1) / STEPS;
  extern __shared__ __attribute__((aligned(16))) char smem[];
  const int lane = threadIdx.x & 63;
  const int wave = __builtin_amdgcn_readfirstlane(threadIdx.x >> 6);

  int tm, tn;
  gemm_tile_coords(xcd_contiguous(blockIdx.x, g.tiles_m * g.tiles_n), g.tiles_m, g.tiles_n, g.gm, tm, tn);
  const int m0 = tm * T::BM, n0 = tn * T::BN;

  int ktiles = 0;
  for (int s = 0; s < g.nseg; ++s) ktiles += g.seg[s].K / BK;

  f32x4 acc[TM][TN];
#pragma unroll
  for (int i = 0; i < TM; ++i)
#pragma unroll
    for (int j = 0; j < TN; ++j) acc[i][j] = (f32x4){0.f, 0.f, 0.f, 0.f};

  const int wr = wave / CFG::WN, wc = wave - wr * CFG::WN;
  const int frow = lane & 15, fq = lane >> 4;

  bf16x8 bh[KS][TN], bl[KS][TN], nbh[KS][TN], nbl[KS][TN], ah[2], al[2];
  ST st;
  if constexpr (BATCH) { st.za = (int64_t)blockIdx.y * g.bs_a; st.zw = (int64_t)blockIdx.y * g.bs_w; }
  st.open_segment(g, 0, m0, n0, wc, wave, lane);
  auto issue_all = [&](char* stage) {
    [&]<int... I>(std::integer_sequence<int, I...>) { (st.template issue<I>(g, stage, wave, nbh, nbl), ...); }(std::make_integer_sequence<int, NOPS>{});
  };
  issue_all(smem);
  st.advance(g, m0, n0, wc, wave, lane);
  asm volatile("s_waitcnt vmcnt(0)" ::: "memory");
  __syncthreads();

  const int arow0 = wr * TM * 16 + frow;
  auto load_a = [&](const char* stage, int ks, int i, bf16x8& h, bf16x8& l) {
    const int row = arow0 + 16 * i;
    const int off = row * (BK * 2) + (((ks * 4 + fq) ^ swz<BK>(row)) << 4);
    h = *reinterpret_cast<const bf16x8*>(stage + off);
    if (TERMS == 3) l = *reinterpret_cast<const bf16x8*>(stage + T::PLANE_A + off);
  };
  auto step = [&](auto s_t, const char* cur, char* nxt, bool has_next) {
    constexpr int s = decltype(s_t)::value, ks = s / TM, i = s % TM;
    if (TERMS == 3) asm volatile("" ::"v"(ah[s & 1]), "v"(al[s & 1]));
    else asm volatile("" ::"v"(ah[s & 1]));
    if constexpr (s + 1 < STEPS) load_a(cur, (s + 1) / TM, (s + 1) % TM, ah[(s + 1) & 1], al[(s + 1) & 1]);
    if (has_next) {
      [&]<int... O>(std::integer_sequence<int, O...>) {
        ([&] {
          constexpr int op = s * OPS_PER_STEP + O;
          if constexpr (op < NOPS) st.template issue<op>(g, nxt, wave, nbh, nbl);
        }(), ...);
      }(std::make_integer_sequence<int, OPS_PER_STEP>{});
    }
    __builtin_amdgcn_sched_barrier(0);
#pragma unroll
    for (int j = 0; j < TN; ++j) {
      if (TERMS == 3) {
        if constexpr (!WX) acc[i][j] = mfma16<F16>(ah[s & 1], bl[ks][j], acc[i][j]);
        acc[i][j] = mfma16<F16>(al[s & 1], bh[ks][j], acc[i][j]);
      }
      acc[i][j] = mfma16<F16>(ah[s & 1], bh[ks][j], acc[i][j]);
    }
    __builtin_amdgcn_sched_barrier(0);
  };

  for (int kt = 0; kt < ktiles; ++kt) {
    const char* cur = smem + (kt & 1) * T::STAGE;
    char* nxt = smem + ((kt + 1) & 1) * T::STAGE;
    const bool has_next = kt + 1 < ktiles;
#pragma unroll
    for (int ks = 0; ks < KS; ++ks)
#pragma unroll
      for (int j = 0; j < TN; ++j) { bh[ks][j] = nbh[ks][j]; if (TERMS == 3 && !WX) bl[ks][j] = nbl[ks][j]; }
    load_a(cur, 0, 0, ah[0], al[0]);
    [&]<int... S>(std::integer_sequence<int, S...>) { (step(std::integral_constant<int, S>{}, cur, nxt, has_next), ...); }(std::make_integer_sequence<int, STEPS>{});
    if (has_next) st.advance(g, m0, n0, wc, wave, lane);
    asm volatile("s_waitcnt vmcnt(0)" ::: "memory");
    __syncthreads();
  }

  static_assert(TN == 4, "epilogue strips are 64 columns wide");
  constexpr int PITCH = 68;
  float* patch = reinterpret_cast<float*>(smem) + wave * (16 * PITCH);
  const int em0 = m0 + wr * TM * 16, en = n0 + wc * 64 + frow * 4;
  float4 bias4 = make_float4(0.f, 0.f, 0.f, 0.f);
  if (g.out.bias && en < g.out.n_valid) bias4 = *reinterpret_cast<const float4*>(g.out.bias + en);
  GemmOut out_z;
  if constexpr (BATCH) { out_z = g.out; out_z.f32 += (int64_t)blockIdx.y * g.bs_o; if (out_z.resid) out_z.resid += (int64_t)blockIdx.y * g.bs_o; }
  const GemmOut& gout = BATCH ? out_z : g.out;
  auto strips = [&](auto full_t) {
    constexpr bool FULL = decltype(full_t)::value;
    float4 side[4], side_next[4];
#pragma unroll
    for (int it = 0; it < 4; ++it) side[it] = load_side4<EPI, FULL>(gout, em0 + fq + 4 * it, en, g.M);
#pragma unroll
    for (int i = 0; i < TM; ++i) {
#pragma unroll
      for (int j = 0; j < TN; ++j)
#pragma unroll
        for (int rr = 0; rr < 4; ++rr) patch[(fq * 4 + rr) * PITCH + j * 16 + frow] = acc[i][j][rr];
      if (i + 1 < TM) {
#pragma unroll
        for (int it = 0; it < 4; ++it) side_next[it] = load_side4<EPI, FULL>(gout, em0 + (i + 1) * 16 + fq + 4 * it, en, g.M);
      }
      __builtin_amdgcn_wave_barrier();
      asm volatile("s_waitcnt lgkmcnt(0)" ::: "memory");
#pragma unroll
      for (int it = 0; it < 4; ++it) {
        const int rl = fq + 4 * it;
        const float4 v = *reinterpret_cast<const float4*>(patch + rl * PITCH + frow * 4);
        store_out4<EPI, F16, FULL>(gout, em0 + i * 16 + rl, en, v, side[it], bias4, g.M);
      }
#pragma unroll
      for (int it = 0; it < 4; ++it) side[it] = side_next[it];
      __builtin_amdgcn_wave_barrier();
      asm volatile("s_waitcnt lgkmcnt(0)" ::: "memory");
    }
  };
  if (m0 + T::BM <= g.M && n0 + T::BN <= g.out.n_valid) strips(std::true_type{}); else strips(std::false_type{});
}


struct CfgF8W4 { static constexpr int WM = 1, WN = 4, TM = 4, TN = 2; };
struct CfgF8Sq { static constexpr int WM = 2, WN = 2, TM = 2, TN = 2; };

template <int OFF>
__device__ __forceinline__ bf16x8 gload16(unsigned voff, const void* sbase) {
  bf16x8 v;
  asm volatile("global_load_dwordx4 %0, %1, %2 offset:%3" : "=v"(v) : "v"(voff), "s"(sbase), "n"(OFF));
  return v;
}
template <int N> __device__ __forceinline__ void wait_vm() { asm volatile("s_waitcnt vmcnt(%0)" ::"n"(N) : "memory"); }
template <int N> __device__ __forceinline__ void wait_vm(bf16x8& f0, bf16x8& f1) { asm volatile("s_waitcnt vmcnt(%2)" : "+v"(f0), "+v"(f1) : "n"(N) : "memory"); }
template <int N> __device__ __forceinline__ void wait_vm8(bf16x8& f0, bf16x8& f1, bf16x8& f2, bf16x8& f3, bf16x8& f4, bf16x8& f5, bf16x8& f6, bf16x8& f7) {
  asm volatile("s_waitcnt vmcnt(%8)" : "+v"(f0), "+v"(f1), "+v"(f2), "+v"(f3), "+v"(f4), "+v"(f5), "+v"(f6), "+v"(f7) : "n"(N) : "memory");
}
template <int N> __device__ __forceinline__ void wait_vm4(bf16x8& f0, bf16x8& f1, bf16x8& f2, bf16x8& f3) {
  asm volatile("s_waitcnt vmcnt(%4)" : "+v"(f0), "+v"(f1), "+v"(f2), "+v"(f3) : "n"(N) : "memory");
}
template <int OFF>
__device__ __forceinline__ bf16x8 lds_read16(unsigned addr) {
  bf16x8 v;
  asm volatile("ds_read_b128 %0, %1 offset:%2" : "=v"(v) : "v"(addr), "n"(OFF));
  return v;
// ... 142 lines not shown
  const unsigned lds0 = (unsigned)(uintptr_t)(__attribute__((address_space(3))) const char*)(smem);
  unsigned a16a[4], a8a[2];
#pragma unroll
  for (int ks = 0; ks < 4; ++ks) a16a[ks] = lds0 + (wr * TM * 32 + r32) * 128 + (((2 * ks + half) ^ ((r32 >> 1) & 7)) << 4);
#pragma unroll
  for (int c = 0; c < 2; ++c) a8a[c] = lds0 + PL16 + (wr * TM * 32 + r32) * 64 + (((2 * half + c) ^ ((r32 >> 2) & 3)) << 4);

  constexpr int DMA_PER_STEP = (NDMA + TM - 1) / TM;
  using ORD = F8IssueOrder<TM, TN, NDMA, NW8>;
  static_assert(ORD::DMA_PER_STEP == DMA_PER_STEP && ORD::NW16 == NW16, "issue-order table and kernel disagree");
  auto ktile = [&](auto pf_t, int kt) {
    constexpr bool PF = decltype(pf_t)::value;
    constexpr int STG = 0;
    char* nxt = smem + ((kt + 1) & 1) * STAGE;
    if constexpr (PF) advance();
    constexpr int AD = MULTI ? 1 : 3;
    bf16x8 af[AD + 1];
    auto read_a16 = [&](auto s_t) {
      constexpr int S2 = decltype(s_t)::value;
      af[S2 % (AD + 1)] = lds_read16<STG * STAGE + (S2 % TM) * 32 * 128>(a16a[S2 / TM]);
    };
    [&]<int... S>(std::integer_sequence<int, S...>) { (read_a16(std::integral_constant<int, S>{}), ...); }(std::make_integer_sequence<int, AD>{});
    bf16x8 ax[2], ay[2];
    auto read_x = [&](auto i_t) { constexpr int O = STG * STAGE + decltype(i_t)::value * 32 * 64; ax[0] = lds_read16<O>(a8a[0]); ax[1] = lds_read16<O>(a8a[1]); };
    auto read_y = [&](auto i_t) { constexpr int O = STG * STAGE + decltype(i_t)::value * 32 * 64 + PL8; ay[0] = lds_read16<O>(a8a[0]); ay[1] = lds_read16<O>(a8a[1]); };
    constexpr bool EARLY8 = !MULTI;
    auto read_yb = [&](auto i_t) {
      constexpr int I = decltype(i_t)::value, O = STG * STAGE + I * 32 * 64 + PL8;
      if constexpr (I & 1) { ax[0] = lds_read16<O>(a8a[0]); ax[1] = lds_read16<O>(a8a[1]); }
      else { ay[0] = lds_read16<O>(a8a[0]); ay[1] = lds_read16<O>(a8a[1]); }
    };
    [&]<int... S>(std::integer_sequence<int, S...>) {
      ([&] {
        constexpr int ks = S / TM, i = S % TM;
        if constexpr (S + AD < 4 * TM) read_a16(std::integral_constant<int, S + AD>{});
        if constexpr (EARLY8 && !WX && S == 4 * TM - 2) read_x(std::integral_constant<int, 0>{});
        if constexpr (EARLY8 && S == 4 * TM - 1) { if constexpr (WX) read_yb(std::integral_constant<int, 0>{}); else read_y(std::integral_constant<int, 0>{}); }
        if constexpr (PF && ks == 0) {
          [&]<int... O>(std::integer_sequence<int, O...>) {
            ([&] { constexpr int op = i * DMA_PER_STEP + O; if constexpr (op < NDMA) dma(std::integral_constant<int, op>{}, nxt); }(), ...);
          }(std::make_integer_sequence<int, DMA_PER_STEP>{});
        }
        constexpr int AHEAD = (4 * TM - 1 - S < AD ? 4 * TM - 1 - S : AD) + (EARLY8 && !WX && S >= 4 * TM - 2 ? 2 : 0) + (EARLY8 && S >= 4 * TM - 1 ? 2 : 0);
        lgkm_wait<AHEAD>(af[S % (AD + 1)]);
        if constexpr (i == 0) wait_vm<ORD::template w16_wait<PF>(ks)>(w16[ks][0], w16[ks][1]);
        __builtin_amdgcn_sched_barrier(0);
#pragma unroll
        for (int j = 0; j < TN; ++j) acc[i][j] = mfma32<true>(af[S % (AD + 1)], w16[ks][j], acc[i][j]);
        __builtin_amdgcn_sched_barrier(0);
        if constexpr (PF && i == TM - 1) load_w16(std::integral_constant<int, ks>{});
      }(), ...);
    }(std::make_integer_sequence<int, 4 * TM>{});
    static_assert(TN == 2, "the tied wait below names the e4m3 W registers of two column tiles");
    if constexpr (WX) wait_vm4<ORD::template w8_wait<PF>()>(w8[0][0], w8[0][1], w8[1][0], w8[1][1]);
    else wait_vm8<ORD::template w8_wait<PF>()>(w8[0][0], w8[0][1], w8[1][0], w8[1][1], wl8[0][0], wl8[0][1], wl8[1][0], wl8[1][1]);
    if constexpr (!EARLY8) { if constexpr (!WX) read_x(std::integral_constant<int, 0>{}); read_y(std::integral_constant<int, 0>{}); }
    [&]<int... I>(std::integer_sequence<int, I...>) {
      ([&] {
        if constexpr (!WX) {
          lgkm_wait<2>(ax[0], ax[1]);
          __builtin_amdgcn_sched_barrier(0);
          const i32x8 a8 = cat8(ax[0], ax[1]);
#pragma unroll
          for (int j = 0; j < TN; ++j) acc[I][j] = mfma32_f8<e8m0(-kF8Act), e8m0(-kF8Wgt - kF8Lo)>(a8, cat8(wl8[j][0], wl8[j][1]), acc[I][j]);
          __builtin_amdgcn_sched_barrier(0);
          if constexpr (I + 1 < TM) read_x(std::integral_constant<int, I + 1>{});
        }
        if constexpr (WX) {
          if constexpr (I + 1 < TM) read_yb(std::integral_constant<int, I + 1>{});
          bf16x8 (&yb)[2] = (I & 1) ? ax : ay;
          lgkm_wait<(I + 1 < TM ? 2 : 0)>(yb[0], yb[1]);
          __builtin_amdgcn_sched_barrier(0);
          const i32x8 al8 = cat8(yb[0], yb[1]);
#pragma unroll
          for (int j = 0; j < TN; ++j) acc[I][j] = mfma32_f8<e8m0(-kF8Act - kF8Lo), e8m0(-kF8Wgt)>(al8, cat8(w8[j][0], w8[j][1]), acc[I][j]);
          __builtin_amdgcn_sched_barrier(0);
        } else {
          lgkm_wait<(I + 1 < TM ? 2 : 0)>(ay[0], ay[1]);
          __builtin_amdgcn_sched_barrier(0);
          const i32x8 al8 = cat8(ay[0], ay[1]);
#pragma unroll
          for (int j = 0; j < TN; ++j) acc[I][j] = mfma32_f8<e8m0(-kF8Act - kF8Lo), e8m0(-kF8Wgt)>(al8, cat8(w8[j][0], w8[j][1]), acc[I][j]);
          __builtin_amdgcn_sched_barrier(0);
          if constexpr (I + 1 < TM) read_y(std::integral_constant<int, I + 1>{});
        }
      }(), ...);
    }(std::make_integer_sequence<int, TM>{});
    if constexpr (PF) {
      load_w8();
      wait_vm<ORD::dma_wait_at_barrier()>();
    }
    asm volatile("s_waitcnt lgkmcnt(0)" ::: "memory");
    __builtin_amdgcn_s_barrier();
    if constexpr (PF) {
      const int flip = (kt & 1) ? -STAGE : STAGE;
#pragma unroll
      for (int ks = 0; ks < 4; ++ks) a16a[ks] += flip;
#pragma unroll
      for (int c = 0; c < 2; ++c) a8a[c] += flip;
    }
  };
  for (int kt = 0; kt + 1 < ktiles; ++kt) ktile(std::true_type{}, kt);
  ktile(std::false_type{}, ktiles - 1);

  static_assert(TN == 2, "epilogue strips are 64 columns wide");
  constexpr int PITCH = 72;
  float* patch = reinterpret_cast<float*>(smem) + wave * (32 * PITCH);
  const int c8 = (lane & 7) * 8, r8 = lane >> 3;
  const int em0 = m0 + wr * TM * 32, en = n0 + wc * 64 + c8;
  float4 b0 = make_float4(0.f, 0.f, 0.f, 0.f), b1 = b0;
  if (g.out.bias && en < g.out.n_valid) { b0 = *reinterpret_cast<const float4*>(g.out.bias + en); b1 = *reinterpret_cast<const float4*>(g.out.bias + en + 4); }
  constexpr bool SIDE = EPI == EPI_F32_RESID || EPI == EPI_F32_GELU_POS || EPI == EPI_BF16_DGELU;
  auto strips = [&](auto full_t) {
    constexpr bool FULL = decltype(full_t)::value;
    float4 side[4][2], side_next[4][2];
    auto load_sides = [&](float4 (&d)[4][2], int i) {
#pragma unroll
      for (int it = 0; it < 4; ++it) {
        d[it][0] = load_side4<EPI, FULL>(g.out, em0 + i * 32 + r8 + 8 * it, en, g.M);
        d[it][1] = load_side4<EPI, FULL>(g.out, em0 + i * 32 + r8 + 8 * it, en + 4, g.M);
      }
    };
    if constexpr (SIDE) load_sides(side, 0);
#pragma unroll
    for (int i = 0; i < TM; ++i) {
#pragma unroll
      for (int j = 0; j < TN; ++j)
#pragma unroll
        for (int rr = 0; rr < 16; ++rr) patch[((rr & 3) + 8 * (rr >> 2) + 4 * half) * PITCH + j * 32 + r32] = acc[i][j][rr];
      __builtin_amdgcn_wave_barrier();
      asm volatile("s_waitcnt lgkmcnt(0)" ::: "memory");
      if constexpr (SIDE) { if (i + 1 < TM) load_sides(side_next, i + 1); }
#pragma unroll
      for (int it = 0; it < 4; ++it) {
        const int rl = r8 + 8 * it;
        const float4 v0 = *reinterpret_cast<const float4*>(patch + rl * PITCH + c8), v1 = *reinterpret_cast<const float4*>(patch + rl * PITCH + c8 + 4);
        store_out8_f8<EPI, FULL>(g.out, em0 + i * 32 + rl, en, v0, v1, side[it][0], side[it][1], b0, b1, g.M);
      }
      if constexpr (SIDE) {
#pragma unroll
        for (int it = 0; it < 4; ++it) { side[it][0] = side_next[it][0]; side[it][1] = side_next[it][1]; }
      }
      __builtin_amdgcn_wave_barrier();
      asm volatile("s_waitcnt lgkmcnt(0)" ::: "memory");
    }
  };
  if (m0 + BM <= g.M && n0 + BN <= g.out.n_valid) strips(std::true_type{}); else strips(std::false_type{});
}

template <int N> __device__ __forceinline__ void wait_vm(bf16x8& f0, bf16x8& f1, bf16x8& f2, bf16x8& f3) {
  asm volatile("s_waitcnt vmcnt(%4)" : "+v"(f0), "+v"(f1), "+v"(f2), "+v"(f3) : "n"(N) : "memory");
}

template <int EPI>
__global__ __launch_bounds__(256, 2) void gemm_f8s_kernel(GemmArgs g) {
  constexpr int TM = 8, TN = 4, KS = 2;
  constexpr int BM = 128, BN = 256, BK = 64, NT = 256;
  constexpr int PL16 = BM * BK * 2, PL8 = BM * BK, STAGE = PL16 + 2 * PL8;
  constexpr int IT16 = PL16 / 16 / NT, IT8 = PL8 / 16 / NT;
  constexpr int NDMA = IT16 + 2 * IT8, NW16 = KS * TN, NW8 = 2 * TN;
  constexpr unsigned kInvalid = 0xFFFFFFFFu;
  extern __shared__ __attribute__((aligned(16))) char smem[];
  const int lane = threadIdx.x & 63;
  const int wave = __builtin_amdgcn_readfirstlane(threadIdx.x >> 6);
  const int tid = wave * 64 + lane;

  int tm, tn;
  gemm_tile_coords(xcd_contiguous(blockIdx.x, g.tiles_m * g.tiles_n), g.tiles_m, g.tiles_n, g.gm, tm, tn);
  const int m0 = tm * BM, n0 = tn * BN;
  const int wc = wave;
  const int r16 = lane & 15, kq = lane >> 4;

  const int ktiles = g.seg[0].K / BK;

  f32x4 acc[TM][TN];
#pragma unroll
  for (int i = 0; i < TM; ++i)
#pragma unroll
    for (int j = 0; j < TN; ++j) acc[i][j] = (f32x4){};

  unsigned a16o[IT16], a8o[IT8];
  const char *a16b, *a8b, *al8b;
  const char *w16b[TN], *w8b[TN];
  const unsigned wl16 = lane * 16, wl32 = lane * 32;
  int kk = 0;
  auto open_streams = [&]() {
    const GemmSeg& sg = g.seg[0];
    const int mb = m0 < g.M ? m0 : g.M - 1;
    const int grp0 = mb / sg.rows_out;
    const int sr0 = (mb - grp0 * sg.rows_out) * sg.row_mul + sg.row_add;
    const int64_t base_row = (int64_t)grp0 * sg.rows_in + (sr0 > 0 ? sr0 : 0);
#pragma unroll
    for (int it = 0; it < IT16; ++it) {
      const int p = it * NT + tid, row = p >> 3, c = (p & 7) ^ ((row >> 1) & 7);
      int m = m0 + row; m = m < g.M ? m : g.M - 1;
      int64_t src;
      a16o[it] = row_map_source(m, sg.rows_out, sg.rows_in, sg.row_mul, sg.row_add, src) ? (unsigned)(((src - base_row) * sg.lda + c * 8) * 2) : kInvalid;
    }
#pragma unroll
    for (int it = 0; it < IT8; ++it) {
      const int p = it * NT + tid, row = p >> 2, c = (p & 3) ^ ((row >> 3) & 1);
      int m = m0 + row; m = m < g.M ? m : g.M - 1;
      int64_t src;
      a8o[it] = row_map_source(m, sg.rows_out, sg.rows_in, sg.row_mul, sg.row_add, src) ? (unsigned)((src - base_row) * sg.lda + c * 16) : kInvalid;
    }
    a16b = (const char*)sg.a_hi + base_row * sg.lda * 2; a8b = (const char*)sg.a8 + base_row * sg.lda; al8b = (const char*)sg.al8 + base_row * sg.lda;
    const int nt0 = (n0 >> 4) + wc * TN;
    const int64_t w16_ts = (int64_t)sg.w_ksteps * 1024;
    const int64_t w8_ts = (int64_t)(sg.w_ksteps / 2) * 2048;
#pragma unroll
    for (int j = 0; j < TN; ++j) {
      w16b[j] = (const char*)sg.ws16 + (nt0 + j) * w16_ts + (int64_t)sg.w_k0 * 1024;
      w8b[j] = (const char*)sg.ws8 + (nt0 + j) * w8_ts + (int64_t)(sg.w_k0 / 2) * 2048;
    }
  };
  auto advance = [&]() {
    if (kk + 1 < ktiles) {
      ++kk;
      a16b += BK * 2; a8b += BK; al8b += BK;
#pragma unroll
      for (int j = 0; j < TN; ++j) { w16b[j] += KS * 1024; w8b[j] += 2048; }
    }
  };
  auto dma = [&](auto op_t, char* stage) {
    constexpr int OP = decltype(op_t)::value;
    if constexpr (OP < IT16) {
      const unsigned o = a16o[OP];
      glds16(o != kInvalid ? (const void*)(a16b + o) : (const void*)g.zeros, stage + (OP * NT + wave * 64) * 16);
    } else if constexpr (OP < IT16 + IT8) {
      const unsigned o = a8o[OP - IT16];
      glds16(o != kInvalid ? (const void*)(a8b + o) : (const void*)g.zeros, stage + PL16 + ((OP - IT16) * NT + wave * 64) * 16);
    } else {
      constexpr int P8 = OP - IT16 - IT8;
      const unsigned o = a8o[P8];
      glds16(o != kInvalid ? (const void*)(al8b + o) : (const void*)g.zeros, stage + PL16 + PL8 + (P8 * NT + wave * 64) * 16);
    }
  };

  bf16x8 w16[KS][TN];
  bf16x8 w8[TN][2];
  auto load_w16 = [&](auto ks_t) {
    constexpr int ks = decltype(ks_t)::value;
#pragma unroll
    for (int j = 0; j < TN; ++j) w16[ks][j] = gload16<ks * 1024>(wl16, w16b[j]);
  };
  auto load_w8 = [&]() {
#pragma unroll
    for (int j = 0; j < TN; ++j) { w8[j][0] = gload16<0>(wl32, w8b[j]); w8[j][1] = gload16<16>(wl32, w8b[j]); }
  };

  open_streams();
  [&]<int... O>(std::integer_sequence<int, O...>) { (dma(std::integral_constant<int, O>{}, smem), ...); }(std::make_integer_sequence<int, NDMA>{});
  load_w16(std::integral_constant<int, 0>{}); load_w16(std::integral_constant<int, 1>{});
  load_w8();
  wait_vm<0>();
  __builtin_amdgcn_s_barrier();

  const unsigned lds0 = (unsigned)(uintptr_t)(__attribute__((address_space(3))) const char*)(smem);
  unsigned a16a[KS], a8a[2];
#pragma unroll
  for (int ks = 0; ks < KS; ++ks) a16a[ks] = lds0 + r16 * 128 + (((4 * ks + kq) ^ ((r16 >> 1) & 7)) << 4);
#pragma unroll
  for (int q = 0; q < 2; ++q) a8a[q] = lds0 + PL16 + (kq >> 1) * PL8 + r16 * 64 + (((2 * (kq & 1) + q) ^ ((r16 >> 3) & 1)) << 4);

  constexpr int DMA_PER_STEP = (NDMA + TM - 1) / TM;
  using ORD = F8IssueOrder<TM, TN, NDMA, NW8, KS>;
  static_assert(ORD::DMA_PER_STEP == DMA_PER_STEP && ORD::NW16 == NW16, "issue-order table and kernel disagree");
  auto ktile = [&](auto pf_t, int kt) {
    constexpr bool PF = decltype(pf_t)::value;
    char* nxt = smem + ((kt + 1) & 1) * STAGE;
    if constexpr (PF) advance();
    constexpr int AD = 3;
    bf16x8 af[AD + 1];
    auto read_a16 = [&](auto s_t) {
      constexpr int S2 = decltype(s_t)::value;
      af[S2 % (AD + 1)] = lds_read16<(S2 % TM) * 16 * 128>(a16a[S2 / TM]);
    };
    [&]<int... S>(std::integer_sequence<int, S...>) { (read_a16(std::integral_constant<int, S>{}), ...); }(std::make_integer_sequence<int, AD>{});
    bf16x8 ax[2], ay[2];
    auto read_8 = [&](auto i_t) {
      constexpr int I = decltype(i_t)::value, O = I * 16 * 64;
      if constexpr (I & 1) { ay[0] = lds_read16<O>(a8a[0]); ay[1] = lds_read16<O>(a8a[1]); }
      else { ax[0] = lds_read16<O>(a8a[0]); ax[1] = lds_read16<O>(a8a[1]); }
    };
    [&]<int... S>(std::integer_sequence<int, S...>) {
      ([&] {
        constexpr int ks = S / TM, i = S % TM;
        if constexpr (S + AD < KS * TM) read_a16(std::integral_constant<int, S + AD>{});
        if constexpr (S == KS * TM - 1) read_8(std::integral_constant<int, 0>{});
        if constexpr (PF && ks == 0) {
          [&]<int... O>(std::integer_sequence<int, O...>) {
            ([&] { constexpr int op = i * DMA_PER_STEP + O; if constexpr (op < NDMA) dma(std::integral_constant<int, op>{}, nxt); }(), ...);
          }(std::make_integer_sequence<int, DMA_PER_STEP>{});
        }
        constexpr int AHEAD = (KS * TM - 1 - S < AD ? KS * TM - 1 - S : AD) + (S >= KS * TM - 1 ? 2 : 0);
        lgkm_wait<AHEAD>(af[S % (AD + 1)]);
        if constexpr (i == 0) wait_vm<ORD::template w16_wait<PF>(ks)>(w16[ks][0], w16[ks][1], w16[ks][2], w16[ks][3]);
        __builtin_amdgcn_sched_barrier(0);
#pragma unroll
        for (int j = 0; j < TN; ++j) acc[i][j] = mfma16<true>(af[S % (AD + 1)], w16[ks][j], acc[i][j]);
        __builtin_amdgcn_sched_barrier(0);
        if constexpr (PF && i == TM - 1) load_w16(std::integral_constant<int, ks>{});
      }(), ...);
    }(std::make_integer_sequence<int, KS * TM>{});
    wait_vm8<ORD::template w8_wait<PF>()>(w8[0][0], w8[0][1], w8[1][0], w8[1][1], w8[2][0], w8[2][1], w8[3][0], w8[3][1]);
    [&]<int... I>(std::integer_sequence<int, I...>) {
      ([&] {
        if constexpr (I + 1 < TM) read_8(std::integral_constant<int, I + 1>{});
        bf16x8 (&cur)[2] = (I & 1) ? ay : ax;
        lgkm_wait<(I + 1 < TM ? 2 : 0)>(cur[0], cur[1]);
        __builtin_amdgcn_sched_barrier(0);
        const i32x8 a8 = cat8(cur[0], cur[1]);
#pragma unroll
        for (int j = 0; j < TN; ++j)
          acc[I][j] = __builtin_amdgcn_mfma_scale_f32_16x16x128_f8f6f4(a8, cat8(w8[j][0], w8[j][1]), acc[I][j], 0, 0, 0, e8m0(-kF8Act), 0, e8m0(-kF8Wgt - kF8Lo));
        __builtin_amdgcn_sched_barrier(0);
      }(), ...);
    }(std::make_integer_sequence<int, TM>{});
    if constexpr (PF) {
      load_w8();
      wait_vm<ORD::dma_wait_at_barrier()>();
    }
    asm volatile("s_waitcnt lgkmcnt(0)" ::: "memory");
    __builtin_amdgcn_s_barrier();
    if constexpr (PF) {
      const int flip = (kt & 1) ? -STAGE : STAGE;
#pragma unroll
      for (int ks = 0; ks < KS; ++ks) a16a[ks] += flip;
#pragma unroll
      for (int q = 0; q < 2; ++q) a8a[q] += flip;
    }
  };
  for (int kt = 0; kt + 1 < ktiles; ++kt) ktile(std::true_type{}, kt);
  ktile(std::false_type{}, ktiles - 1);

  constexpr int PITCH = 72;
  float* patch = reinterpret_cast<float*>(smem) + wave * (32 * PITCH);
  const int c8 = (lane & 7) * 8, r8 = lane >> 3;
  const int em0 = m0, en = n0 + wc * 64 + c8;
  float4 b0 = make_float4(0.f, 0.f, 0.f, 0.f), b1 = b0;
  if (g.out.bias && en < g.out.n_valid) { b0 = *reinterpret_cast<const float4*>(g.out.bias + en); b1 = *reinterpret_cast<const float4*>(g.out.bias + en + 4); }
  constexpr bool SIDE = EPI == EPI_F32_RESID || EPI == EPI_F32_GELU_POS || EPI == EPI_BF16_DGELU;
  auto strips = [&](auto full_t) {
    constexpr bool FULL = decltype(full_t)::value;
    float4 side[4][2], side_next[4][2];
    auto load_sides = [&](float4 (&d)[4][2], int i) {
#pragma unroll
      for (int it = 0; it < 4; ++it) {
        d[it][0] = load_side4<EPI, FULL>(g.out, em0 + i * 32 + r8 + 8 * it, en, g.M);
        d[it][1] = load_side4<EPI, FULL>(g.out, em0 + i * 32 + r8 + 8 * it, en + 4, g.M);
      }
    };
    if constexpr (SIDE) load_sides(side, 0);
#pragma unroll
    for (int i = 0; i < TM / 2; ++i) {
#pragma unroll
      for (int rt = 0; rt < 2; ++rt)
#pragma unroll
        for (int ct = 0; ct < TN; ++ct)
#pragma unroll
          for (int reg = 0; reg < 4; ++reg) patch[(rt * 16 + 4 * kq + reg) * PITCH + ct * 16 + r16] = acc[2 * i + rt][ct][reg];
      __builtin_amdgcn_wave_barrier();
      asm volatile("s_waitcnt lgkmcnt(0)" ::: "memory");
      if constexpr (SIDE) { if (i + 1 < TM / 2) load_sides(side_next, i + 1); }
#pragma unroll
      for (int it = 0; it < 4; ++it) {
        const int rl = r8 + 8 * it;
        const float4 v0 = *reinterpret_cast<const float4*>(patch + rl * PITCH + c8), v1 = *reinterpret_cast<const float4*>(patch + rl * PITCH + c8 + 4);
        store_out8_f8<EPI, FULL>(g.out, em0 + i * 32 + rl, en, v0, v1, side[it][0], side[it][1], b0, b1, g.M);
      }
      if constexpr (SIDE) {
#pragma unroll
        for (int it = 0; it < 4; ++it) { side[it][0] = side_next[it][0]; side[it][1] = side_next[it][1]; }
      }
      __builtin_amdgcn_wave_barrier();
      asm volatile("s_waitcnt lgkmcnt(0)" ::: "memory");
    }
  };
  if (m0 + BM <= g.M && n0 + BN <= g.out.n_valid) strips(std::true_type{}); else strips(std::false_type{});
}

template <auto Kernel>
int launch_tiles(GemmArgs a, int bm, int bn, int threads, int lds, hipStream_t s, int batch = 1) {
  a.tiles_m = (a.M + bm - 1) / bm;
  a.tiles_n = (a.N + bn - 1) / bn;
  a.gm = g_gm;
  return launch_kernel<Kernel>(dim3(a.tiles_m * a.tiles_n, batch), dim3(threads), lds, s, a);
}

int g_mfma16 = 1;
template <int EPI>
int launch_f8s(GemmArgs a, hipStream_t s) {
  return launch_tiles<gemm_f8s_kernel<EPI>>(a, 128, 256, 256, 2 * (128 * 64 * 2 + 2 * 128 * 64), s);
}

template <int EPI, class CFG>
int launch_f8(GemmArgs a, hipStream_t s) {
  constexpr int BM = CFG::WM * CFG::TM * 32, BN = CFG::WN * CFG::TN * 32, NT = CFG::WM * CFG::WN * 64;
  constexpr int lds = 2 * (BM * 64 * 2 + 2 * BM * 64);
  if (a.nseg == 1 && a.seg[0].w_exact16) return launch_tiles<gemm_f8_kernel<EPI, CFG, false, true>>(a, BM, BN, NT, lds, s);
  if (a.nseg == 1) return launch_tiles<gemm_f8_kernel<EPI, CFG, false>>(a, BM, BN, NT, lds, s);
  return launch_tiles<gemm_f8_kernel<EPI, CFG, true>>(a, BM, BN, NT, lds, s);
}

template <int EPI, bool ILV>
__global__ __launch_bounds__(512, 2) void gemm_pp_kernel(pp::Args g, GemmOut out) {
  extern __shared__ __attribute__((aligned(16))) char smem[];
  const int lane = threadIdx.x & 63;
  const int wave = __builtin_amdgcn_readfirstlane(threadIdx.x >> 6);
  const int wr = wave >> 2, wc = wave & 3, r16 = lane & 15, kq = lane >> 4;
  float* patch = reinterpret_cast<float*>(smem + pp::PATCH_BASE + wave * 8192);
  const int c8 = (lane & 7) * 8, r8 = lane >> 3;
  constexpr bool SIDE = EPI == EPI_F32_RESID;
  pp::kloop(g, smem, [&](int tm, int tn, pp::Acc& accs) {
    auto& acc = accs.t;
    const int m0 = tm * pp::BM, n0 = tn * pp::BN;
    const int em0 = m0 + wr * 128, en = n0 + wc * 64 + c8;
    float4 b0 = make_float4(0.f, 0.f, 0.f, 0.f), b1 = b0;
    if (out.bias && en < out.n_valid) { b0 = *reinterpret_cast<const float4*>(out.bias + en); b1 = *reinterpret_cast<const float4*>(out.bias + en + 4); }
    auto strips = [&](auto full_t) {
      constexpr bool FULL = decltype(full_t)::value;
      float4 side[4][2], side_next[4][2];
      auto load_sides = [&](float4 (&d)[4][2], int i) {
#pragma unroll
        for (int it = 0; it < 4; ++it) {
          d[it][0] = load_side4<EPI, FULL>(out, em0 + i * 32 + r8 + 8 * it, en, g.M);
          d[it][1] = load_side4<EPI, FULL>(out, em0 + i * 32 + r8 + 8 * it, en + 4, g.M);
        }
      };
      if constexpr (SIDE) load_sides(side, 0);
#pragma unroll
      for (int i = 0; i < 4; ++i) {
#pragma unroll
        for (int rt = 0; rt < 2; ++rt)
#pragma unroll
          for (int ct = 0; ct < 4; ++ct)
#pragma unroll
            for (int reg = 0; reg < 4; ++reg) {
              const int row = rt * 16 + 4 * kq + reg;
              patch[row * 64 + (((ct * 16 + r16 + 16 * kq) & 63) ^ ((reg & 1) << 2))] = acc[2 * i + rt][ct][reg];
            }
        __builtin_amdgcn_wave_barrier();
        asm volatile("s_waitcnt lgkmcnt(0)" ::: "memory");
        if constexpr (SIDE) { if (i + 1 < 4) load_sides(side_next, i + 1); }
#pragma unroll
        for (int it = 0; it < 4; ++it) {
          const int rl = r8 + 8 * it, sw = (rl & 1) << 2, rot = 16 * ((rl >> 2) & 3);
          const float4 v0 = *reinterpret_cast<const float4*>(patch + rl * 64 + (((c8 + rot) & 63) ^ sw)), v1 = *reinterpret_cast<const float4*>(patch + rl * 64 + (((c8 + 4 + rot) & 63) ^ sw));
          store_out8_f8<EPI, FULL, ILV>(out, em0 + i * 32 + rl, en, v0, v1, side[it][0], side[it][1], b0, b1, g.M);
        }
        if constexpr (SIDE) {
#pragma unroll
          for (int it = 0; it < 4; ++it) { side[it][0] = side_next[it][0]; side[it][1] = side_next[it][1]; }
        }
        __builtin_amdgcn_wave_barrier();
        asm volatile("s_waitcnt lgkmcnt(0)" ::: "memory");
      }
    };
    if (m0 + pp::BM <= g.M && n0 + pp::BN <= out.n_valid) strips(std::true_type{}); else strips(std::false_type{});
  });
}

template <int EPI, bool ILV>
int launch_pp(const pp::Args& a, const GemmOut& o, int grid, hipStream_t s) {
  return launch_kernel<gemm_pp_kernel<EPI, ILV>>(dim3(grid), dim3(pp::NT), pp::LDS_BYTES, s, a, o);
}

int g_force_tile = 0;

template <int TERMS, int BK, int EPI, class CFG, bool F16, bool WX, bool BATCH>
int launch_one(GemmArgs a, hipStream_t s, int batch) {
  using T = Tile<TERMS, BK, CFG, WX>;
  return launch_tiles<gemm_kernel<TERMS, BK, EPI, CFG, F16, WX, BATCH>>(a, T::BM, T::BN, T::THREADS, T::LDS_BYTES, s, batch);
}
template <int TERMS, int EPI, bool F16, bool WX = false, bool BATCH = false>
int launch_tile(int tile, GemmArgs a, hipStream_t s, int batch = 1) {
  constexpr int BK = TERMS == 1 ? 64 : 32;
  if (tile == 256) return launch_one<TERMS, BK, EPI, CfgW4, F16, WX, BATCH>(a, s, batch);
  if (tile == 128) return launch_one<TERMS, BK, EPI, Cfg128, F16, WX, BATCH>(a, s, batch);
  return launch_one<TERMS, 64, EPI, Cfg64, F16, WX, BATCH>(a, s, batch);
}

constexpr int kSlots = 512;
int pick_tile(int M, int N, int batch = 1) {
  const int64_t panels = (int64_t)((M + 127) / 128) * batch;
  int tile = g_force_tile;
  if (!tile) tile = (N % 256 == 0 && panels * (N / 256) >= kSlots) ? 256 : (panels * (N / 128) >= kSlots ? 128 : 64);
  return (tile == 256 && N % 256 != 0) ? 128 : tile;
}

template <int EPI>
int launch_epi(GemmArgs a, int prec, hipStream_t s) {
  const int Mp = a.out.m_pick > 0 ? a.out.m_pick : a.M;
  if (prec == PREC_F16F8) {
    const int n256 = (a.N + 255) / 256 * 256;
    const bool f8s_ok = g_mfma16 && a.nseg == 1 && a.seg[0].ws16 && a.seg[0].ws8 && a.seg[0].a8 && !a.seg[0].w_exact16 &&
                        (a.N % 256 == 0 || (a.seg[0].ws_rows >= n256 && (int64_t)n256 * 3 <= (int64_t)a.N * 4));
    const int64_t t256f = (int64_t)((Mp + 127) / 128) * (f8s_ok ? n256 / 256 : a.N / 256);
    int tile = g_force_tile;
    if (!tile) tile = ((a.N % 256 == 0 || f8s_ok) && t256f >= kSlots) ? 256 : 128;
    if (tile == 256 && f8s_ok) return launch_f8s<EPI>(a, s);
    if (tile == 256 && a.N % 256 == 0) return launch_f8<EPI, CfgF8W4>(a, s);
    return launch_f8<EPI, CfgF8Sq>(a, s);
  }
  const int tile = pick_tile(Mp, a.N);
  if (prec == PREC_F16X3) {
    return (a.nseg == 1 && a.seg[0].w_exact16) ? launch_tile<3, EPI, true, true>(tile, a, s) : launch_tile<3, EPI, true>(tile, a, s);
  }
  if (prec == PREC_F16) return launch_tile<1, EPI, true>(tile, a, s);
  return prec_products(prec) == 3 ? launch_tile<3, EPI, false>(tile, a, s) : launch_tile<1, EPI, false>(tile, a, s);
}


template <int EPI>
int launch_batched_epi(GemmArgs a, int batch, hipStream_t s) {
  const int tail = a.M % 128;
  const int tile = (!g_force_tile && tail > 0 && tail <= 64 && a.M < 1024) ? 64 : pick_tile(a.M, a.N, batch);
  return launch_tile<3, EPI, false, false, true>(tile, a, s, batch);
}

}

int launch_gemm_batched(awt_ctx* c, int batch, int M, int N, int K, const bf16_t* a_hi, const bf16_t* a_lo, int64_t lda, int64_t bs_a, const bf16_t* w_hi,
                        const bf16_t* w_lo, int64_t bs_w, float* out, const float* resid, int64_t ldo, int64_t bs_o, int n_valid, hipStream_t s) {
  AWT_REQUIRE(c && c->zeros && batch > 0 && batch <= 65535 && M > 0 && N > 0 && N % 128 == 0 && K > 0 && K % 64 == 0, AWT_ERR_INVALID,
              "gemm (batched): 1..65535 matrices, N % 128 == 0 and K % 64 == 0 required");
  AWT_REQUIRE(a_hi && a_lo && w_hi && w_lo && out && lda % 8 == 0 && lda >= K && ldo % 4 == 0 && n_valid > 0 && n_valid <= N && n_valid % 4 == 0 && ldo >= n_valid, AWT_ERR_INVALID,
              "gemm (batched): null plane, lda not a multiple of 8, or output columns / pitch not a multiple of 4");
  AWT_REQUIRE(bs_a % 8 == 0 && bs_w % 8 == 0 && bs_o % 4 == 0, AWT_ERR_INVALID, "gemm (batched): matrix strides must keep 16-byte alignment");
  GemmArgs a{};
  a.M = M; a.N = N; a.nseg = 1; a.zeros = (const bf16_t*)c->zeros;
  GemmSeg& sg = a.seg[0];
  sg.a_hi = a_hi; sg.a_lo = a_lo; sg.lda = lda; sg.w_hi = w_hi; sg.w_lo = w_lo; sg.w_ksteps = K / 32; sg.w_k0 = 0; sg.K = K;
  sg.rows_out = sg.rows_in = M; sg.row_mul = 1; sg.row_add = 0;
  a.out.f32 = out; a.out.resid = resid; a.out.ldo = ldo; a.out.n_valid = n_valid;
  a.bs_a = bs_a; a.bs_w = bs_w; a.bs_o = bs_o;
  ProfScope prof(c, AWT_PROF_GEMM, s, 2.0 * (double)batch * (double)M * (double)n_valid * (double)K);
  return resid ? launch_batched_epi<EPI_F32_RESID>(a, batch, s) : launch_batched_epi<EPI_F32>(a, batch, s);
}

int g_pp_mode = 1;
int awt_gemm_pp_mode() { return g_pp_mode; }
void awt_gemm_set_pp_mode(int v) { g_pp_mode = v; }
int gemm_pp_slots() {
  static int n_cu[64] = {};
  int dev = 0;
  if (hipGetDevice(&dev) != hipSuccess) return 0;
  if (!n_cu[dev & 63]) { hipDeviceProp_t p; if (hipGetDeviceProperties(&p, dev) != hipSuccess) return 0; n_cu[dev & 63] = p.multiProcessorCount > 0 ? p.multiProcessorCount : 256; }
  return n_cu[dev & 63];
}
bool gemm_pp_supported(int M, int N, int K, int epi) {
  return M > 0 && N > 0 && N % 256 == 0 && K >= 128 && K % 64 == 0 &&
         (epi == EPI_F32 || epi == EPI_F32_RESID || epi == EPI_BF16 || epi == EPI_BF16_GELU || epi == EPI_QKV);
}
int launch_gemm_pp(awt_ctx* c, int M, int N, const GemmSeg& seg, GemmEpilogue epi, const GemmOut& out, hipStream_t s) {
  AWT_REQUIRE(c && gemm_pp_supported(M, N, seg.K, epi), AWT_ERR_INVALID, "gemm (ping-pong): N % 256 == 0, K % 64 == 0, K >= 128 and a supported epilogue required");
  AWT_REQUIRE(seg.a_ilv && seg.w_pp && seg.rows_out == M && seg.rows_in == M && seg.row_mul == 1 && seg.row_add == 0 && seg.w_k0 == 0 && seg.w_ksteps == seg.K / 32 && seg.lda == seg.K,
              AWT_ERR_INVALID, "gemm (ping-pong): one plain, dense K segment over split-line activations and a packed weight image");
  AWT_REQUIRE(!out.ilv || ((epi == EPI_BF16 || epi == EPI_BF16_GELU) && out.ldo == N && out.n_valid == N), AWT_ERR_INVALID, "gemm (ping-pong): a split-line output is a dense [M, N] activation");
  pp::Args a{};
  a.A = seg.a_ilv; a.a_row_bytes = (int64_t)seg.lda * 4; a.W = seg.w_pp;
  a.M = M; a.N = N; a.K = seg.K; a.nk = seg.K / 32;
  a.tiles_m = (M + pp::BM - 1) / pp::BM; a.tiles_n = N / pp::BN; a.ntiles = a.tiles_m * a.tiles_n; a.gm = g_gm;
  const int grid = std::min(a.ntiles, gemm_pp_slots());
  ProfScope prof(c, AWT_PROF_GEMM, s, 2.0 * (double)M * (double)out.n_valid * (double)seg.K);
  switch (epi) {
    case EPI_F32: return launch_pp<EPI_F32, false>(a, out, grid, s);
    case EPI_F32_RESID: return launch_pp<EPI_F32_RESID, false>(a, out, grid, s);
    case EPI_BF16: return out.ilv ? launch_pp<EPI_BF16, true>(a, out, grid, s) : launch_pp<EPI_BF16, false>(a, out, grid, s);
    case EPI_BF16_GELU: return out.ilv ? launch_pp<EPI_BF16_GELU, true>(a, out, grid, s) : launch_pp<EPI_BF16_GELU, false>(a, out, grid, s);
    case EPI_QKV: return launch_pp<EPI_QKV, false>(a, out, grid, s);
    default: break;
  }
  return awt_fail(AWT_ERR_INVALID, "gemm (ping-pong): unsupported epilogue");
}

void awt_gemm_set_mfma16(int v) { g_mfma16 = v; }
void awt_gemm_force_tile(int t) { g_force_tile = t; }
void awt_gemm_set_gm(int v) { g_gm = v > 0 ? v : AWT_GEMM_GM; }

int launch_gemm(awt_ctx* c, int M, int N, const GemmSeg* segs, int nseg, int prec, GemmEpilogue epi, const GemmOut& out,
                hipStream_t s) {
  AWT_REQUIRE(M > 0 && N > 0 && N % 128 == 0, AWT_ERR_INVALID, "gemm: N must be a positive multiple of 128");
  AWT_REQUIRE(nseg >= 1 && nseg <= kMaxSeg, AWT_ERR_INVALID, "gemm: 1..3 K-segments");
  AWT_REQUIRE(prec_known(prec), AWT_ERR_INVALID, "gemm: unknown operand precision");
  const int terms = prec_products(prec);
  AWT_REQUIRE(c && c->zeros, AWT_ERR_INVALID, "gemm: context without a zero page");
  GemmArgs a{};
  a.M = M; a.N = N; a.nseg = nseg; a.out = out; a.zeros = (const bf16_t*)c->zeros;
  double ksum = 0;
  for (int i = 0; i < nseg; ++i) {
    a.seg[i] = segs[i];
    AWT_REQUIRE(segs[i].K > 0 && segs[i].K % 64 == 0, AWT_ERR_INVALID, "gemm: every K-segment must be a positive multiple of 64");
    if (prec == PREC_F16F8) AWT_REQUIRE(segs[i].a_hi && segs[i].w_hi && (segs[i].a8 || (segs[i].w_exact16 && nseg == 1)) && segs[i].al8 && segs[i].w8 && segs[i].wl8 && segs[i].w_ksteps % 2 == 0 && segs[i].w_k0 % 2 == 0,
                                        AWT_ERR_INVALID, "gemm (f16f8): null operand plane or a K-segment that is not 64-aligned in its weight matrix");
    else AWT_REQUIRE(segs[i].a_hi && segs[i].w_hi && (terms == 1 || (segs[i].a_lo && segs[i].w_lo)), AWT_ERR_INVALID, "gemm: null operand plane");
    AWT_REQUIRE(segs[i].lda % 8 == 0 && segs[i].w_ksteps > 0 && segs[i].w_k0 >= 0 && segs[i].w_k0 + segs[i].K / 32 <= segs[i].w_ksteps, AWT_ERR_INVALID,
                "gemm: lda must be a multiple of 8 and the segment must lie inside its fragment-major weight matrix");
    AWT_REQUIRE(segs[i].rows_out > 0 && segs[i].rows_in > 0 && segs[i].row_mul > 0 && (int64_t)segs[i].row_mul * segs[i].rows_out == segs[i].rows_in, AWT_ERR_INVALID,
                "gemm: bad row map (rows_in must be row_mul * rows_out)");
    ksum += segs[i].K;
  }
  ProfScope prof(c, AWT_PROF_GEMM, s, 2.0 * (double)M * (double)out.n_valid * ksum);
  switch (epi) {
    case EPI_F32: return launch_epi<EPI_F32>(a, prec, s);
    case EPI_F32_RESID: return launch_epi<EPI_F32_RESID>(a, prec, s);
    case EPI_BF16: return launch_epi<EPI_BF16>(a, prec, s);
    case EPI_BF16_GELU: return launch_epi<EPI_BF16_GELU>(a, prec, s);
    case EPI_QKV: return launch_epi<EPI_QKV>(a, prec, s);
    case EPI_F32_GELU_POS: return launch_epi<EPI_F32_GELU_POS>(a, prec, s);
    case EPI_BF16_GELU_SAVE: return launch_epi<EPI_BF16_GELU_SAVE>(a, prec, s);
    case EPI_BF16_DGELU: return launch_epi<EPI_BF16_DGELU>(a, prec, s);
  }
  return awt_fail(AWT_ERR_INVALID, "gemm: unknown epilogue");
}
```

Baseline: 1437 clips/s.

## Fuse LayerNorm into residual GEMM epilogues via last-arriving-tile panel counters

Adds a fused LayerNorm path to the residual fp32 GEMMs (out_proj and fc2). Each output tile increments a per-row-panel atomic counter, and the last tile to arrive for a 128-row panel normalizes those rows. It writes the next consumer's operand directly: ln2 after out_proj, the next layer's ln1 after fc2, or the final layer_norm. This removes separate layernorm launches and their extra fp32 round trip, and the LayerNorm code is factored into a shared header. The cost is acquire/release fences, a serialized tail of work in the last-arriving block, and persistent counters that must be reset correctly.

```diff
diff --git a/mlx8-ws-audio-transformer_amd/build.py b/mlx8-ws-audio-transformer_amd/build.py
--- a/mlx8-ws-audio-transformer_amd/build.py
+++ b/mlx8-ws-audio-transformer_amd/build.py
@@ -23,7 +23,7 @@
 
 def _compile(src: str, force: bool) -> str:
     obj = os.path.join(OBJ, src.replace(".hip", ".o"))
-    deps = [os.path.join(CSRC, src), os.path.join(CSRC, "common.h"), os.path.join(CSRC, "comm.h"), os.path.join(CSRC, "gemm_pp.h"), os.path.join(CSRC, "wgrad.h"), os.path.join(HERE, "..", "include", "awt.h")]
+    deps = [os.path.join(CSRC, src), os.path.join(CSRC, "common.h"), os.path.join(CSRC, "comm.h"), os.path.join(CSRC, "gemm_pp.h"), os.path.join(CSRC, "wgrad.h"), os.path.join(CSRC, "layernorm_row.h"), os.path.join(CSRC, "panel_arrival.h"), os.path.join(HERE, "..", "include", "awt.h")]
     if force or _stale(obj, deps):
         cmd = [HIPCC, *FLAGS, "-c", os.path.join(CSRC, src), "-o", obj]
         r = subprocess.run(cmd, capture_output=True, text=True)
diff --git a/mlx8-ws-audio-transformer_amd/csrc/awt_api.hip b/mlx8-ws-audio-transformer_amd/csrc/awt_api.hip
--- a/mlx8-ws-audio-transformer_amd/csrc/awt_api.hip
+++ b/mlx8-ws-audio-transformer_amd/csrc/awt_api.hip
@@ -37,6 +37,7 @@
 }
 
 static int g_conv_live = 1;
+static int g_ln_fuse = 3;
 static int g_pp_mask = 12;
 extern "C" int awt_tuning_set(const char* key, int value) {
   AWT_REQUIRE(key, AWT_ERR_INVALID, "tuning_set: null key");
@@ -58,6 +59,11 @@
   if (!strcmp(key, "gemm_pp_mask")) {
     AWT_REQUIRE(value >= 0 && value <= 15, AWT_ERR_INVALID, "tuning_set: gemm_pp_mask is a bit set 0 .. 15 (1 qkv, 2 out_proj, 4 fc1, 8 fc2; fc2 only together with fc1)");
     g_pp_mask = value;
+    return AWT_OK;
+  }
+  if (!strcmp(key, "ln_fuse")) {
+    AWT_REQUIRE(value >= 0 && value <= 3, AWT_ERR_INVALID, "tuning_set: ln_fuse is a bit set 0 .. 3 (1 out_proj -> ln2, 2 fc2 -> the next ln1 / the final layer_norm)");
+    g_ln_fuse = value;
     return AWT_OK;
   }
   if (!strcmp(key, "gemm_mfma16")) {
@@ -124,11 +130,29 @@
     delete c;
     AWT_REQUIRE(false, AWT_ERR_HIP, "ctx_create: could not allocate the zero page");
   }
+  c->ln_cnt_n = 1024;
+  if (hipMalloc((void**)&c->ln_cnt, c->ln_cnt_n * sizeof(unsigned)) != hipSuccess || hipMemset(c->ln_cnt, 0, c->ln_cnt_n * sizeof(unsigned)) != hipSuccess) {
+    (void)hipFree(c->zeros);
+    delete c;
+    AWT_REQUIRE(false, AWT_ERR_HIP, "ctx_create: could not allocate the panel counters");
+  }
   int rc = logmel_prepare_impl(c, 400, 80, 0.0, 8000.0, 16000, 1);
   if (!rc) rc = logmel_prepare_impl(c, 400, 128, 0.0, 8000.0, 16000, 1);
   if (rc) { awt_ctx_destroy(c); return rc; }
   *out = c;
   return AWT_OK;
+}
+unsigned* awt_ln_counters(awt_ctx* c, int panels, hipStream_t s) {
+  if (panels <= c->ln_cnt_n) return c->ln_cnt;
+  hipStreamCaptureStatus st = hipStreamCaptureStatusNone;
+  if (hipStreamIsCapturing(s, &st) != hipSuccess || st != hipStreamCaptureStatusNone) return nullptr;
+  const int n = (panels + 1023) / 1024 * 1024;
+  unsigned* p = nullptr;
+  if (hipDeviceSynchronize() != hipSuccess || hipMalloc((void**)&p, n * sizeof(unsigned)) != hipSuccess) return nullptr;
+  if (hipMemset(p, 0, n * sizeof(unsigned)) != hipSuccess || hipDeviceSynchronize() != hipSuccess) { (void)hipFree(p); return nullptr; }
+  (void)hipFree(c->ln_cnt);
+  c->ln_cnt = p; c->ln_cnt_n = n;
+  return p;
 }
 extern "C" int awt_logmel_prepare(awt_ctx* c, int n_fft, int n_mels, float f_min, float f_max, int sample_rate, int slaney) {
   return logmel_prepare_impl(c, n_fft, n_mels, (double)f_min, (double)f_max, sample_rate, slaney);
@@ -138,6 +162,7 @@
   if (!c) return;
   awt_free_tables(c);
   if (c->zeros) (void)hipFree(c->zeros);
+  if (c->ln_cnt) (void)hipFree(c->ln_cnt);
   if (c->prof) {
     for (int k = 0; k < AWT_PROF_NCLASSES; ++k)
       for (auto& sp : c->prof->spans[k]) { (void)hipEventDestroy(sp.a); (void)hipEventDestroy(sp.b); }
@@ -474,7 +499,8 @@
   return launch_expand_conv_rows(e->ctx, g, e->pos, Bc, S, Sc, d, x, s);
 }
 
-int encoder_layer(awt_encoder* e, Layer& L, const LayerBufs& b, int Bc, bool save, hipStream_t s) {
+int encoder_layer(awt_encoder* e, Layer& L, const LayerBufs& b, int Bc, bool save, hipStream_t s, bool ln1_done = false, const Layer* next = nullptr,
+                  float* final_hidden = nullptr, bool* next_ln_done = nullptr) {
   const awt_encoder_cfg& c = e->cfg;
   const int S = c.n_ctx, d = c.d_model, f = c.ffn_dim, H = c.n_heads, terms = e->prec;
   const int M = Bc * S;
@@ -484,8 +510,15 @@
   auto feeds = [&](Act a, const Linear& lin, const LoraGroup& lg) { if (terms == PREC_F16F8 && lin.w.exact16 && !lg.active) a.hi8 = nullptr; return a; };
   const Act aqkv = make_act(b.qkv[0], b.qkv[1], 3 * (size_t)plane, terms);
   const Act aatt = pp_out ? make_ilv(b.att[0]) : feeds(make_act(b.att[0], b.att[1], (size_t)plane, terms), L.out, L.lo_);
-  int rc = launch_layernorm(e->ctx, b.x_in, L.ln1_g, L.ln1_b, M, d, 1e-5f, nullptr,
-                            pp_qkv ? make_ilv(b.ln1[0]) : feeds(make_act(b.ln1[0], b.ln1[1], (size_t)plane, terms), L.qkv, L.lq), terms, s); if (rc) return rc;
+  auto ln1_dest = [&](const Layer& X) {
+    const bool ppq = !save && (g_pp_mask & 1) && use_pp(e, X.qkv, X.lq, M, EPI_QKV);
+    return ppq ? make_ilv(b.ln1[0]) : feeds(make_act(b.ln1[0], b.ln1[1], (size_t)plane, terms), X.qkv, X.lq);
+  };
+  const bool fuse_ln2 = !save && (g_ln_fuse & 1) && terms == PREC_F16F8 && !L.lo_.active;
+  const bool fuse_next = !save && (g_ln_fuse & 2) && terms == PREC_F16F8 && !L.l2.active && (next || final_hidden);
+  if (next_ln_done) *next_ln_done = fuse_next;
+  int rc = AWT_OK;
+  if (!ln1_done) { rc = launch_layernorm(e->ctx, b.x_in, L.ln1_g, L.ln1_b, M, d, 1e-5f, nullptr, ln1_dest(L), terms, s); if (rc) return rc; }
   {
     GemmOut o{}; set_out(o, aqkv); o.scale = 0.125f * 1.4426950408889634f;
     o.S = S; o.H = H; o.plane_stride = plane;
@@ -504,6 +537,10 @@
   if (rc) return rc;
   {
     GemmOut o{}; o.f32 = b.x_mid; o.resid = b.x_in; o.ldo = d;
+    if (fuse_ln2) {
+      o.ln_g = L.ln2_g; o.ln_b = L.ln2_b; o.ln_eps = 1e-5f;
+      o.ln_act = pp_fc1 ? make_ilv(b.ln2[0]) : feeds(make_act(b.ln2[0], b.ln2[1], (size_t)plane, terms), L.fc1, L.l1);
+    }
     rc = pp_out ? linear_pp(e, b.att[0], L.out, M, EPI_F32_RESID, o, s) : linear_with_lora(e, b.uo, b.att, d, L.out, L.lo_, M, EPI_F32_RESID, o, s);
     if (rc) return rc;
   }
@@ -517,8 +554,10 @@
     GemmOut o2{}; o2.f32 = b.x_out; o2.resid = b.x_mid; o2.ldo = d; o2.n_valid = d; o2.bias = L.fc2.bias;
     return launch_gemm(e->ctx, M, d, &s2, 1, PREC_F16F8, EPI_F32_RESID, o2, s);
   }
-  rc = launch_layernorm(e->ctx, b.x_mid, L.ln2_g, L.ln2_b, M, d, 1e-5f, nullptr,
-                        pp_fc1 ? make_ilv(b.ln2[0]) : feeds(make_act(b.ln2[0], b.ln2[1], (size_t)plane, terms), L.fc1, L.l1), terms, s); if (rc) return rc;
+  if (!fuse_ln2) {
+    rc = launch_layernorm(e->ctx, b.x_mid, L.ln2_g, L.ln2_b, M, d, 1e-5f, nullptr,
+                          pp_fc1 ? make_ilv(b.ln2[0]) : feeds(make_act(b.ln2[0], b.ln2[1], (size_t)plane, terms), L.fc1, L.l1), terms, s); if (rc) return rc;
+  }
   {
     GemmOut o{}; set_out(o, pp_fc2 ? make_ilv(b.ff[0]) : feeds(make_act(b.ff[0], b.ff[1], (size_t)M * f, terms), L.fc2, L.l2)); o.ldo = f; o.hi2 = b.pre[0]; o.lo2 = b.pre[1];
     rc = pp_fc1 ? linear_pp(e, b.ln2[0], L.fc1, M, EPI_BF16_GELU, o, s)
@@ -526,6 +565,11 @@
     if (rc) return rc;
   }
   GemmOut o{}; o.f32 = b.x_out; o.resid = b.x_mid; o.ldo = d;
+  if (fuse_next) {
+    o.ln_eps = 1e-5f;
+    if (next) { o.ln_g = next->ln1_g; o.ln_b = next->ln1_b; o.ln_act = ln1_dest(*next); }
+    else { o.ln_g = e->lnf_g; o.ln_b = e->lnf_b; o.ln_f32 = final_hidden; }
+  }
   return pp_fc2 ? linear_pp(e, b.ff[0], L.fc2, M, EPI_F32_RESID, o, s) : linear_with_lora(e, b.u2, b.ff, f, L.fc2, L.l2, M, EPI_F32_RESID, o, s);
 }
 
@@ -555,7 +599,12 @@
     b.ln1[p] = b.ln2[p] = on ? w.ln[p] : nullptr; b.qkv[p] = on ? w.qkv[p] : nullptr; b.att[p] = on ? w.att[p] : nullptr;
     b.ff[p] = on ? w.ff[p] : nullptr; b.u[p] = b.uo[p] = b.u1[p] = b.u2[p] = on ? w.u[p] : nullptr; b.pre[p] = nullptr;
   }
-  for (int li = 0; li < c.n_layers; ++li) { rc = encoder_layer(e, e->layers[li], b, Bc, false, s); if (rc) return rc; }
+  bool ln_done = false;
+  for (int li = 0; li < c.n_layers; ++li) {
+    const bool is_last = li + 1 == c.n_layers;
+    rc = encoder_layer(e, e->layers[li], b, Bc, false, s, ln_done, is_last ? nullptr : &e->layers[li + 1], is_last ? hidden : nullptr, &ln_done); if (rc) return rc;
+  }
+  if (ln_done) return AWT_OK;
   return launch_layernorm(e->ctx, w.x, e->lnf_g, e->lnf_b, M, d, 1e-5f, hidden, Act{}, e->prec, s);
 }
 
diff --git a/mlx8-ws-audio-transformer_amd/csrc/common.h b/mlx8-ws-audio-transformer_amd/csrc/common.h
--- a/mlx8-ws-audio-transformer_amd/csrc/common.h
+++ b/mlx8-ws-audio-transformer_amd/csrc/common.h
@@ -250,7 +250,10 @@
   struct Table;
   Table* tables = nullptr;
   void* zeros = nullptr;
-};
+  unsigned* ln_cnt = nullptr;
+  int ln_cnt_n = 0;
+};
+unsigned* awt_ln_counters(awt_ctx* c, int panels, hipStream_t s);
 
 #define AWT_ONCE_PER_DEVICE(set)                                   \
   do {                                                             \
@@ -327,6 +330,9 @@
   int64_t plane_stride;
   int skip_v8;
   int m_pick;
+  const float* ln_g; const float* ln_b; float ln_eps;
+  float* ln_f32; Act ln_act;
+  unsigned* ln_cnt; int ln_tiles;
 };
 
 int launch_gemm(awt_ctx* c, int M, int N, const GemmSeg* segs, int nseg, int prec, GemmEpilogue epi, const GemmOut& out,
diff --git a/mlx8-ws-audio-transformer_amd/csrc/elementwise.hip b/mlx8-ws-audio-transformer_amd/csrc/elementwise.hip
--- a/mlx8-ws-audio-transformer_amd/csrc/elementwise.hip
+++ b/mlx8-ws-audio-transformer_amd/csrc/elementwise.hip
@@ -1,14 +1,8 @@
 #include "common.h"
 #include "gemm_pp.h"
+#include "layernorm_row.h"
 
 namespace {
-
-__device__ __forceinline__ float4 ldg_once(const float4* p) {
-  const f32x4 t = __builtin_nontemporal_load(reinterpret_cast<const f32x4*>(p));
-  return make_float4(t[0], t[1], t[2], t[3]);
-}
-
-constexpr int kLnMaxChunks = 5;
 
 template <int PREC>
 __global__ __launch_bounds__(256) void layernorm_kernel(const float* __restrict__ x, const float* __restrict__ gamma,
@@ -17,44 +11,9 @@
   const int lane = threadIdx.x & 63;
   const int row = blockIdx.x * 4 + (threadIdx.x >> 6);
   if (row >= M) return;
-  const int nchunk = d >> 2;
-  const float4* xr = reinterpret_cast<const float4*>(x + (int64_t)row * d);
   float4 v[kLnMaxChunks];
-  float sum = 0.f;
-#pragma unroll
-  for (int i = 0; i < kLnMaxChunks; ++i) {
-    const int c = lane + 64 * i;
-    if (c < nchunk) v[i] = ldg_once(xr + c);
-    else v[i] = make_float4(0.f, 0.f, 0.f, 0.f);
-    sum += (v[i].x + v[i].y) + (v[i].z + v[i].w);
-  }
-#pragma unroll
-  for (int o = 32; o > 0; o >>= 1) sum += __shfl_xor(sum, o);
-  const float mean = sum / (float)d;
-  float sq = 0.f;
-#pragma unroll
-  for (int i = 0; i < kLnMaxChunks; ++i) {
-    const int c = lane + 64 * i;
-    if (c < nchunk) {
-      const float a = v[i].x - mean, b = v[i].y - mean, cc = v[i].z - mean, dd = v[i].w - mean;
-      sq += (a * a + b * b) + (cc * cc + dd * dd);
-    }
-  }
-#pragma unroll
-  for (int o = 32; o > 0; o >>= 1) sq += __shfl_xor(sq, o);
-  const float rstd = 1.0f / sqrtf(sq / (float)d + eps);
-  const float4* g4 = reinterpret_cast<const float4*>(gamma);
-  const float4* b4 = reinterpret_cast<const float4*>(beta);
-#pragma unroll
-  for (int i = 0; i < kLnMaxChunks; ++i) {
-    const int c = lane + 64 * i;
-    if (c >= nchunk) continue;
-    const float4 g = g4[c], bb = b4[c];
-    float y[4] = {(v[i].x - mean) * rstd * g.x + bb.x, (v[i].y - mean) * rstd * g.y + bb.y,
-                  (v[i].z - mean) * rstd * g.z + bb.z, (v[i].w - mean) * rstd * g.w + bb.w};
-    if (out_f32) reinterpret_cast<float4*>(out_f32 + (int64_t)row * d)[c] = make_float4(y[0], y[1], y[2], y[3]);
-    else store_act4<PREC>(out, (int64_t)row * d + 4 * c, y);
-  }
+  ln_row_load<kLnMaxChunks, true>(x, row, d, lane, v);
+  ln_row_finish<PREC, kLnMaxChunks>(v, gamma, beta, row, d, eps, lane, out_f32, out);
 }
 
 __global__ __launch_bounds__(256) void split_kernel(const float* __restrict__ x, int64_t n4, float scale, bf16_t* hi, bf16_t* lo) {
diff --git a/mlx8-ws-audio-transformer_amd/csrc/gemm.hip b/mlx8-ws-audio-transformer_amd/csrc/gemm.hip
--- a/mlx8-ws-audio-transformer_amd/csrc/gemm.hip
+++ b/mlx8-ws-audio-transformer_amd/csrc/gemm.hip
@@ -2,6 +2,8 @@
 #include <type_traits>
 #include "common.h"
 #include "gemm_pp.h"
+#include "layernorm_row.h"
+#include "panel_arrival.h"
 
 #ifndef AWT_GEMM_GM
 #define AWT_GEMM_GM 8
@@ -177,7 +179,10 @@
   }
 }
 
-template <int EPI, bool FULL, bool ILV = false>
+__device__ __forceinline__ void store16_sc1(float* p, f32x4 v) {
+  asm volatile("global_store_dwordx4 %0, %1, off sc1\n\ts_nop 1" ::"v"(p), "v"(v) : "memory");
+}
+template <int EPI, bool FULL, bool ILV = false, bool SC1 = false>
 __device__ __forceinline__ void store_out8_f8(const GemmOut& o, int m, int n, float4 acc0, float4 acc1, float4 side0, float4 side1, float4 b0, float4 b1, int M) {
   if constexpr (!FULL) { if (m >= M || n >= o.n_valid) return; }
   float v[8] = {acc0.x, acc0.y, acc0.z, acc0.w, acc1.x, acc1.y, acc1.z, acc1.w};
@@ -187,6 +192,11 @@
     float* dst = o.f32 + (int64_t)m * o.ldo + n;
 #pragma unroll
     for (int t = 0; t < 8; ++t) v[t] = EPI == EPI_F32_RESID ? v[t] + sd[t] : (EPI == EPI_F32_GELU_POS ? gelu_erf(v[t]) + sd[t] : v[t]);
+    if constexpr (SC1) {
+      store16_sc1(dst, (f32x4){v[0], v[1], v[2], v[3]});
+      store16_sc1(dst + 4, (f32x4){v[4], v[5], v[6], v[7]});
+      return;
+    }
     *reinterpret_cast<float4*>(dst) = make_float4(v[0], v[1], v[2], v[3]);
     *reinterpret_cast<float4*>(dst + 4) = make_float4(v[4], v[5], v[6], v[7]);
     return;
@@ -242,6 +252,23 @@
   if (EPI == EPI_QKV && o.skip_v8 && n >= 2 * o.H * 64) return;
   if (o.hi8) __builtin_nontemporal_store((i32x2){(int)fp8x4_rt(v[0], v[1], v[2], v[3], lim8, inv8), (int)fp8x4_rt(v[4], v[5], v[6], v[7], lim8, inv8)}, reinterpret_cast<i32x2*>(o.hi8 + off));
   __builtin_nontemporal_store((i32x2){(int)fp8x4_rt(l[0], l[1], l[2], l[3], liml8, invl8), (int)fp8x4_rt(l[4], l[5], l[6], l[7], liml8, invl8)}, reinterpret_cast<i32x2*>(o.lo8 + off));
+}
+
+#if defined(AWT_LNF_SC1)
+constexpr bool kLnfSc1 = true;
+#else
+constexpr bool kLnfSc1 = false;
+#endif
+__device__ __forceinline__ void ln_close_panel(const GemmOut& o, unsigned* cnt, int64_t row0, int rows, int d, int wave, int nwaves, int lane) {
+  if (d == 768 && (o.ln_f32 || o.ln_act.ilv || o.ln_act.hi8)) {
+    const int nfull = rows & ~7;
+    if (o.ln_f32) ln_rows_exact<LN_DEST_F32, 3, 8>(o.f32, o.ln_g, o.ln_b, row0, nfull, o.ln_eps, wave, nwaves, lane, o.ln_f32, o.ln_act);
+    else if (o.ln_act.ilv) ln_rows_exact<LN_DEST_ILV, 3, 8>(o.f32, o.ln_g, o.ln_b, row0, nfull, o.ln_eps, wave, nwaves, lane, o.ln_f32, o.ln_act);
+    else ln_rows_exact<LN_DEST_PLANES, 3, 8>(o.f32, o.ln_g, o.ln_b, row0, nfull, o.ln_eps, wave, nwaves, lane, o.ln_f32, o.ln_act);
+    ln_rows<PREC_F16F8, 3, 1>(o.f32, o.ln_g, o.ln_b, row0 + nfull, rows - nfull, d, o.ln_eps, wave, nwaves, lane, o.ln_f32, o.ln_act);
+  } else if (d <= 768) ln_rows<PREC_F16F8, 3, 2>(o.f32, o.ln_g, o.ln_b, row0, rows, d, o.ln_eps, wave, nwaves, lane, o.ln_f32, o.ln_act);
+  else ln_rows<PREC_F16F8, kLnMaxChunks, 2>(o.f32, o.ln_g, o.ln_b, row0, rows, d, o.ln_eps, wave, nwaves, lane, o.ln_f32, o.ln_act);
+  if (wave == 0 && lane == 0) panel_reset(cnt);
 }
 
 template <int TERMS, int BK, int EPI, class CFG, bool F16, bool WX = false, bool BATCH = false>
@@ -690,8 +717,9 @@
   asm volatile("s_waitcnt vmcnt(%4)" : "+v"(f0), "+v"(f1), "+v"(f2), "+v"(f3) : "n"(N) : "memory");
 }
 
-template <int EPI>
+template <int EPI, bool LNF = false>
 __global__ __launch_bounds__(256, 2) void gemm_f8s_kernel(GemmArgs g) {
+  static_assert(!LNF || EPI == EPI_F32_RESID, "the fused LayerNorm reads the fp32 output of the residual epilogue");
   constexpr int TM = 8, TN = 4, KS = 2;
   constexpr int BM = 128, BN = 256, BK = 64, NT = 256;
   constexpr int PL16 = BM * BK * 2, PL8 = BM * BK, STAGE = PL16 + 2 * PL8;
@@ -905,7 +933,7 @@
       for (int it = 0; it < 4; ++it) {
         const int rl = r8 + 8 * it;
         const float4 v0 = *reinterpret_cast<const float4*>(patch + rl * PITCH + c8), v1 = *reinterpret_cast<const float4*>(patch + rl * PITCH + c8 + 4);
-        store_out8_f8<EPI, FULL>(g.out, em0 + i * 32 + rl, en, v0, v1, side[it][0], side[it][1], b0, b1, g.M);
+        store_out8_f8<EPI, FULL, false, LNF && kLnfSc1>(g.out, em0 + i * 32 + rl, en, v0, v1, side[it][0], side[it][1], b0, b1, g.M);
       }
       if constexpr (SIDE) {
 #pragma unroll
@@ -916,6 +944,17 @@
     }
   };
   if (m0 + BM <= g.M && n0 + BN <= g.out.n_valid) strips(std::true_type{}); else strips(std::false_type{});
+
+  if constexpr (LNF) {
+    asm volatile("s_waitcnt vmcnt(0)" ::: "memory");
+    __syncthreads();
+    int* const last = reinterpret_cast<int*>(smem);
+    unsigned* const cnt = g.out.ln_cnt + tm;
+    if (tid == 0) *last = panel_arrive(cnt, (unsigned)g.out.ln_tiles) ? 1 : 0;
+    __syncthreads();
+    if (__builtin_amdgcn_readfirstlane(*last) == 0) return;
+    ln_close_panel(g.out, cnt, m0, min(BM, g.M - m0), g.N, wave, NT / 64, lane);
+  }
 }
 
 template <auto Kernel>
@@ -929,6 +968,9 @@
 int g_mfma16 = 1;
 template <int EPI>
 int launch_f8s(GemmArgs a, hipStream_t s) {
+  if constexpr (EPI == EPI_F32_RESID) {
+    if (a.out.ln_cnt) return launch_tiles<gemm_f8s_kernel<EPI, true>>(a, 128, 256, 256, 2 * (128 * 64 * 2 + 2 * 128 * 64), s);
+  }
   return launch_tiles<gemm_f8s_kernel<EPI>>(a, 128, 256, 256, 2 * (128 * 64 * 2 + 2 * 128 * 64), s);
 }
 
@@ -941,8 +983,9 @@
   return launch_tiles<gemm_f8_kernel<EPI, CFG, true>>(a, BM, BN, NT, lds, s);
 }
 
-template <int EPI, bool ILV>
+template <int EPI, bool ILV, bool LNF = false>
 __global__ __launch_bounds__(512, 2) void gemm_pp_kernel(pp::Args g, GemmOut out) {
+  static_assert(!LNF || EPI == EPI_F32_RESID, "the fused LayerNorm reads the fp32 output of the residual epilogue");
   extern __shared__ __attribute__((aligned(16))) char smem[];
   const int lane = threadIdx.x & 63;
   const int wave = __builtin_amdgcn_readfirstlane(threadIdx.x >> 6);
@@ -985,7 +1028,7 @@
         for (int it = 0; it < 4; ++it) {
           const int rl = r8 + 8 * it, sw = (rl & 1) << 2, rot = 16 * ((rl >> 2) & 3);
           const float4 v0 = *reinterpret_cast<const float4*>(patch + rl * 64 + (((c8 + rot) & 63) ^ sw)), v1 = *reinterpret_cast<const float4*>(patch + rl * 64 + (((c8 + 4 + rot) & 63) ^ sw));
-          store_out8_f8<EPI, FULL, ILV>(out, em0 + i * 32 + rl, en, v0, v1, side[it][0], side[it][1], b0, b1, g.M);
+          store_out8_f8<EPI, FULL, ILV, LNF && kLnfSc1>(out, em0 + i * 32 + rl, en, v0, v1, side[it][0], side[it][1], b0, b1, g.M);
         }
         if constexpr (SIDE) {
 #pragma unroll
@@ -996,12 +1039,23 @@
       }
     };
     if (m0 + pp::BM <= g.M && n0 + pp::BN <= out.n_valid) strips(std::true_type{}); else strips(std::false_type{});
+    if constexpr (LNF) {
+      asm volatile("s_waitcnt vmcnt(0)" ::: "memory");
+      __builtin_amdgcn_s_barrier();
+      int* const last = reinterpret_cast<int*>(smem + pp::PATCH_BASE);
+      unsigned* const cnt = out.ln_cnt + tm;
+      if (wave == 0 && lane == 0) *last = panel_arrive(cnt, (unsigned)out.ln_tiles) ? 1 : 0;
+      asm volatile("s_waitcnt lgkmcnt(0)" ::: "memory");
+      __builtin_amdgcn_s_barrier();
+      asm volatile("" ::: "memory");
+      if (__builtin_amdgcn_readfirstlane(*last) != 0) ln_close_panel(out, cnt, m0, min(pp::BM, g.M - m0), g.N, wave, pp::NT / 64, lane);
+    }
   });
 }
 
-template <int EPI, bool ILV>
+template <int EPI, bool ILV, bool LNF = false>
 int launch_pp(const pp::Args& a, const GemmOut& o, int grid, hipStream_t s) {
-  return launch_kernel<gemm_pp_kernel<EPI, ILV>>(dim3(grid), dim3(pp::NT), pp::LDS_BYTES, s, a, o);
+  return launch_kernel<gemm_pp_kernel<EPI, ILV, LNF>>(dim3(grid), dim3(pp::NT), pp::LDS_BYTES, s, a, o);
 }
 
 int g_force_tile = 0;
@@ -1027,21 +1081,28 @@
   return (tile == 256 && N % 256 != 0) ? 128 : tile;
 }
 
+int f8_route(const GemmArgs& a) {
+  const int Mp = a.out.m_pick > 0 ? a.out.m_pick : a.M;
+  const int n256 = (a.N + 255) / 256 * 256;
+  const bool f8s_ok = g_mfma16 && a.nseg == 1 && a.seg[0].ws16 && a.seg[0].ws8 && a.seg[0].a8 && !a.seg[0].w_exact16 &&
+                      (a.N % 256 == 0 || (a.seg[0].ws_rows >= n256 && (int64_t)n256 * 3 <= (int64_t)a.N * 4));
+  const int64_t t256f = (int64_t)((Mp + 127) / 128) * (f8s_ok ? n256 / 256 : a.N / 256);
+  int tile = g_force_tile;
+  if (!tile) tile = ((a.N % 256 == 0 || f8s_ok) && t256f >= kSlots) ? 256 : 128;
+  if (tile == 256 && f8s_ok) return 0;
+  if (tile == 256 && a.N % 256 == 0) return 1;
+  return 2;
+}
+
 template <int EPI>
 int launch_epi(GemmArgs a, int prec, hipStream_t s) {
-  const int Mp = a.out.m_pick > 0 ? a.out.m_pick : a.M;
   if (prec == PREC_F16F8) {
-    const int n256 = (a.N + 255) / 256 * 256;
-    const bool f8s_ok = g_mfma16 && a.nseg == 1 && a.seg[0].ws16 && a.seg[0].ws8 && a.seg[0].a8 && !a.seg[0].w_exact16 &&
-                        (a.N % 256 == 0 || (a.seg[0].ws_rows >= n256 && (int64_t)n256 * 3 <= (int64_t)a.N * 4));
-    const int64_t t256f = (int64_t)((Mp + 127) / 128) * (f8s_ok ? n256 / 256 : a.N / 256);
-    int tile = g_force_tile;
-    if (!tile) tile = ((a.N % 256 == 0 || f8s_ok) && t256f >= kSlots) ? 256 : 128;
-    if (tile == 256 && f8s_ok) return launch_f8s<EPI>(a, s);
-    if (tile == 256 && a.N % 256 == 0) return launch_f8<EPI, CfgF8W4>(a, s);
+    const int route = f8_route(a);
+    if (route == 0) return launch_f8s<EPI>(a, s);
+    if (route == 1) return launch_f8<EPI, CfgF8W4>(a, s);
     return launch_f8<EPI, CfgF8Sq>(a, s);
   }
-  const int tile = pick_tile(Mp, a.N);
+  const int tile = pick_tile(a.out.m_pick > 0 ? a.out.m_pick : a.M, a.N);
   if (prec == PREC_F16X3) {
     return (a.nseg == 1 && a.seg[0].w_exact16) ? launch_tile<3, EPI, true, true>(tile, a, s) : launch_tile<3, EPI, true>(tile, a, s);
   }
@@ -1077,6 +1138,14 @@
   return resid ? launch_batched_epi<EPI_F32_RESID>(a, batch, s) : launch_batched_epi<EPI_F32>(a, batch, s);
 }
 
+static bool ln_request_ok(const GemmOut& o, int N, int prec, int epi) {
+  return epi == EPI_F32_RESID && o.f32 && o.ln_b && o.ldo == N && o.n_valid == N && N % 4 == 0 && N <= 64 * 4 * kLnMaxChunks &&
+         (o.ln_f32 || (prec == PREC_F16F8 ? (o.ln_act.ilv ? N % 64 == 0 : o.ln_act.p16 && o.ln_act.lo8) : o.ln_act.p16 != nullptr));
+}
+static int ln_after(awt_ctx* c, const GemmOut& o, int M, int N, int prec, hipStream_t s) {
+  return launch_layernorm(c, o.f32, o.ln_g, o.ln_b, M, N, o.ln_eps, o.ln_f32, o.ln_act, prec, s);
+}
+
 int g_pp_mode = 1;
 int awt_gemm_pp_mode() { return g_pp_mode; }
 void awt_gemm_set_pp_mode(int v) { g_pp_mode = v; }
@@ -1101,6 +1170,14 @@
   a.M = M; a.N = N; a.K = seg.K; a.nk = seg.K / 32;
   a.tiles_m = (M + pp::BM - 1) / pp::BM; a.tiles_n = N / pp::BN; a.ntiles = a.tiles_m * a.tiles_n; a.gm = g_gm;
   const int grid = std::min(a.ntiles, gemm_pp_slots());
+  if (out.ln_g) {
+    AWT_REQUIRE(ln_request_ok(out, N, PREC_F16F8, epi), AWT_ERR_INVALID, "gemm (ping-pong): a fused LayerNorm needs the residual epilogue, a dense fp32 output of at most 1280 columns and a destination");
+    GemmOut o = out;
+    o.ln_cnt = awt_ln_counters(c, a.tiles_m, s); o.ln_tiles = a.tiles_n;
+    if (!o.ln_cnt) { o.ln_g = nullptr; const int rc = launch_gemm_pp(c, M, N, seg, epi, o, s); return rc ? rc : ln_after(c, out, M, N, PREC_F16F8, s); }
+    ProfScope prof(c, AWT_PROF_GEMM, s, 2.0 * (double)M * (double)out.n_valid * (double)seg.K);
+    return launch_pp<EPI_F32_RESID, false, true>(a, o, grid, s);
+  }
   ProfScope prof(c, AWT_PROF_GEMM, s, 2.0 * (double)M * (double)out.n_valid * (double)seg.K);
   switch (epi) {
     case EPI_F32: return launch_pp<EPI_F32, false>(a, out, grid, s);
@@ -1139,6 +1216,17 @@
                 "gemm: bad row map (rows_in must be row_mul * rows_out)");
     ksum += segs[i].K;
   }
+  if (out.ln_g) {
+    AWT_REQUIRE(ln_request_ok(out, N, prec, epi), AWT_ERR_INVALID, "gemm: a fused LayerNorm needs the residual epilogue, a dense fp32 output of at most 1280 columns and a destination");
+    a.out.ln_cnt = nullptr;
+    if (prec == PREC_F16F8 && N % 256 == 0 && f8_route(a) == 0) { a.out.ln_cnt = awt_ln_counters(c, (M + 127) / 128, s); a.out.ln_tiles = N / 256; }
+    int rc;
+    {
+      ProfScope prof(c, AWT_PROF_GEMM, s, 2.0 * (double)M * (double)out.n_valid * ksum);
+      rc = launch_epi<EPI_F32_RESID>(a, prec, s);
+    }
+    return rc || a.out.ln_cnt ? rc : ln_after(c, out, M, N, prec, s);
+  }
   ProfScope prof(c, AWT_PROF_GEMM, s, 2.0 * (double)M * (double)out.n_valid * ksum);
   switch (epi) {
     case EPI_F32: return launch_epi<EPI_F32>(a, prec, s);
diff --git a/mlx8-ws-audio-transformer_amd/csrc/layernorm_row.h b/mlx8-ws-audio-transformer_amd/csrc/layernorm_row.h
--- /dev/null
+++ b/mlx8-ws-audio-transformer_amd/csrc/layernorm_row.h
@@ -0,0 +1,125 @@
+#pragma once
+#include "common.h"
+
+constexpr int kLnMaxChunks = 5;
+
+__device__ __forceinline__ float4 ldg_once(const float4* p) {
+  const f32x4 t = __builtin_nontemporal_load(reinterpret_cast<const f32x4*>(p));
+  return make_float4(t[0], t[1], t[2], t[3]);
+}
+
+template <int MAXC, bool ONCE>
+__device__ __forceinline__ void ln_row_load(const float* x, int64_t row, int d, int lane, float4 (&v)[MAXC]) {
+  const int nchunk = d >> 2;
+  const float4* xr = reinterpret_cast<const float4*>(x + row * d);
+#pragma unroll
+  for (int i = 0; i < MAXC; ++i) {
+    const int c = lane + 64 * i;
+    if (c < nchunk) v[i] = ONCE ? ldg_once(xr + c) : xr[c];
+    else v[i] = make_float4(0.f, 0.f, 0.f, 0.f);
+  }
+}
+
+template <int MAXC, bool EXACT>
+__device__ __forceinline__ void ln_row_stats(const float4 (&v)[MAXC], int d, float eps, int lane, float& mean, float& rstd) {
+#pragma clang fp contract(off)
+  const int nchunk = d >> 2;
+  float sum = 0.f;
+#pragma unroll
+  for (int i = 0; i < MAXC; ++i) sum += (v[i].x + v[i].y) + (v[i].z + v[i].w);
+#pragma unroll
+  for (int i = MAXC; i < kLnMaxChunks; ++i) sum += 0.f;
+#pragma unroll
+  for (int o = 32; o > 0; o >>= 1) sum += __shfl_xor(sum, o);
+  mean = sum / (float)d;
+  float sq = 0.f;
+#pragma unroll
+  for (int i = 0; i < MAXC; ++i) {
+    const int c = lane + 64 * i;
+    if (EXACT || c < nchunk) {
+      const float a = v[i].x - mean, b = v[i].y - mean, cc = v[i].z - mean, dd = v[i].w - mean;
+      sq += __builtin_fmaf(a, a, b * b) + __builtin_fmaf(cc, cc, dd * dd);
+    }
+  }
+#pragma unroll
+  for (int o = 32; o > 0; o >>= 1) sq += __shfl_xor(sq, o);
+  rstd = 1.0f / sqrtf(sq / (float)d + eps);
+}
+__device__ __forceinline__ void ln_affine4(const float4& v, float mean, float rstd, const float4& g, const float4& bb, float (&y)[4]) {
+#pragma clang fp contract(off)
+  y[0] = __builtin_fmaf((v.x - mean) * rstd, g.x, bb.x); y[1] = __builtin_fmaf((v.y - mean) * rstd, g.y, bb.y);
+  y[2] = __builtin_fmaf((v.z - mean) * rstd, g.z, bb.z); y[3] = __builtin_fmaf((v.w - mean) * rstd, g.w, bb.w);
+}
+
+template <int PREC, int MAXC>
+__device__ __forceinline__ void ln_row_finish(const float4 (&v)[MAXC], const float* gamma, const float* beta, int64_t row, int d, float eps, int lane,
+                                              float* out_f32, const Act& out) {
+  const int nchunk = d >> 2;
+  float mean, rstd;
+  ln_row_stats<MAXC, false>(v, d, eps, lane, mean, rstd);
+  const float4* g4 = reinterpret_cast<const float4*>(gamma);
+  const float4* b4 = reinterpret_cast<const float4*>(beta);
+#pragma unroll
+  for (int i = 0; i < MAXC; ++i) {
+    const int c = lane + 64 * i;
+    if (c >= nchunk) continue;
+    float y[4];
+    ln_affine4(v[i], mean, rstd, g4[c], b4[c], y);
+    if (out_f32) reinterpret_cast<float4*>(out_f32 + row * d)[c] = make_float4(y[0], y[1], y[2], y[3]);
+    else store_act4<PREC>(out, row * d + 4 * c, y);
+  }
+}
+
+template <int PREC, int MAXC, int RB>
+__device__ __forceinline__ void ln_rows(const float* x, const float* gamma, const float* beta, int64_t row0, int nrows, int d, float eps, int wave,
+                                        int nwaves, int lane, float* out_f32, const Act& out) {
+  for (int r = wave * RB; r < nrows; r += nwaves * RB) {
+    float4 v[RB][MAXC];
+#pragma unroll
+    for (int j = 0; j < RB; ++j)
+      if (r + j < nrows) ln_row_load<MAXC, false>(x, row0 + r + j, d, lane, v[j]);
+#pragma unroll
+    for (int j = 0; j < RB; ++j)
+      if (r + j < nrows) ln_row_finish<PREC, MAXC>(v[j], gamma, beta, row0 + r + j, d, eps, lane, out_f32, out);
+  }
+}
+
+enum { LN_DEST_F32 = 0, LN_DEST_PLANES = 1, LN_DEST_ILV = 2 };
+template <int DEST, int MAXC, int RB>
+__device__ __forceinline__ void ln_rows_exact(const float* x, const float* gamma, const float* beta, int64_t row0, int nrows, float eps, int wave, int nwaves,
+                                              int lane, float* out_f32, const Act& out) {
+  constexpr int d = 256 * MAXC;
+  float4 g[MAXC], bb[MAXC];
+#pragma unroll
+  for (int i = 0; i < MAXC; ++i) { g[i] = reinterpret_cast<const float4*>(gamma)[lane + 64 * i]; bb[i] = reinterpret_cast<const float4*>(beta)[lane + 64 * i]; }
+  for (int r = wave * RB; r < nrows; r += nwaves * RB) {
+    float4 v[RB][MAXC];
+#pragma unroll
+    for (int j = 0; j < RB; ++j) ln_row_load<MAXC, false>(x, row0 + r + j, d, lane, v[j]);
+#pragma unroll
+    for (int j = 0; j < RB; ++j) {
+      float mean, rstd;
+      ln_row_stats<MAXC, true>(v[j], d, eps, lane, mean, rstd);
+      const int64_t row = row0 + r + j;
+#pragma unroll
+      for (int i = 0; i < MAXC; ++i) {
+        const int c = lane + 64 * i;
+        float y[4];
+        ln_affine4(v[j][i], mean, rstd, g[i], bb[i], y);
+        const int64_t off = row * d + 4 * c;
+        if constexpr (DEST == LN_DEST_F32) {
+          *reinterpret_cast<float4*>(out_f32 + off) = make_float4(y[0], y[1], y[2], y[3]);
+        } else {
+          uint2 h16; unsigned hi8, lo8;
+          f16f8x4<kF8Act, false>(y, h16, hi8, lo8);
+          if constexpr (DEST == LN_DEST_ILV) store_ilv4(out.ilv, off, h16, hi8, lo8);
+          else {
+            *reinterpret_cast<uint2*>(out.p16 + off) = h16;
+            *reinterpret_cast<unsigned*>(out.hi8 + off) = hi8;
+            *reinterpret_cast<unsigned*>(out.lo8 + off) = lo8;
+          }
+        }
+      }
+    }
+  }
+}
diff --git a/mlx8-ws-audio-transformer_amd/csrc/panel_arrival.h b/mlx8-ws-audio-transformer_amd/csrc/panel_arrival.h
--- /dev/null
+++ b/mlx8-ws-audio-transformer_amd/csrc/panel_arrival.h
@@ -0,0 +1,34 @@
+#pragma once
+
+#if defined(__HIPCC__)
+#include <hip/hip_runtime.h>
+#define AWT_ARRIVAL_FN __host__ __device__ inline
+#else
+#define AWT_ARRIVAL_FN inline
+#endif
+
+AWT_ARRIVAL_FN bool panel_arrive(unsigned* cnt, unsigned tiles) {
+#if defined(__HIP_DEVICE_COMPILE__)
+#if !defined(AWT_LNF_SC1) && !defined(AWT_LNF_NO_RELEASE)
+  __builtin_amdgcn_fence(__ATOMIC_RELEASE, "agent");
+  asm volatile("s_waitcnt vmcnt(0)" ::: "memory");
+#endif
+  const unsigned old = __hip_atomic_fetch_add(cnt, 1u, __ATOMIC_RELAXED, __HIP_MEMORY_SCOPE_AGENT);
+  const bool last = old + 1u == tiles;
+  if (last) {
+    __builtin_amdgcn_fence(__ATOMIC_ACQUIRE, "agent");
+    asm volatile("s_waitcnt vmcnt(0)" ::: "memory");
+  }
+  return last;
+#else
+  return __atomic_fetch_add(cnt, 1u, __ATOMIC_ACQ_REL) + 1u == tiles;
+#endif
+}
+
+AWT_ARRIVAL_FN void panel_reset(unsigned* cnt) {
+#if defined(__HIP_DEVICE_COMPILE__)
+  __hip_atomic_store(cnt, 0u, __ATOMIC_RELAXED, __HIP_MEMORY_SCOPE_AGENT);
+#else
+  __atomic_store_n(cnt, 0u, __ATOMIC_RELEASE);
+#endif
+}
```

Result: slower. 1296 clips/s (-9.8%).
